# shadimsaleh/motion_detection

Measured on AMD Instinct MI355X. Metric: Mpixels/s (flow+warp+diff) at 1080p & 4K; % HBM roofline, 1/2/4/8 GPU, higher is better.
Workload: dtype u8

## Files before the change

motion_detection_amd/csrc/mdx_api.cpp:

```cpp
#include "mdx_ctx.h"

#include <cstdlib>
#include <map>
#include <mutex>

using namespace mdx;

static thread_local std::string g_create_err;

extern "C" void mdx_default_params(mdx_params* p)
{
    p->win = 40;
    p->max_level = 5;
    p->max_iters = 10;
    p->eps = 0.03;
    p->min_eig = 0.001f;
    p->thresh = 190;
    p->pixel_step = 10;
    p->min_vector_size = 1.0;
    p->fit_mode = MDX_FIT_FIRST4;
    p->subspace_precision = MDX_SUBSPACE_F64;
    p->call_pipelining = 0;
    p->ransac_iters = 128;
    p->ransac_thresh = 3.0;
    p->ransac_seed = 20141105u;
}

extern "C" int mdx_grid_count(int w, int h, int ps)
{
    if (w <= 0 || h <= 0 || ps <= 0) return 0;
    return ((w + ps - 1) / ps) * ((h + ps - 1) / ps);
}

static const char* check_params(const mdx_params* p)
{
    if (p->win != kWin) return "only win == 40 (the reference constant) is supported";
    if (p->max_level < 0 || p->max_level >= kMaxLevels) return "max_level out of range [0, 7]";
    if (p->pixel_step <= 0) return "pixel_step must be > 0 (reference leaves it unset: UB)";
    if (p->fit_mode != MDX_FIT_FIRST4 && p->fit_mode != MDX_FIT_EXTERNAL && p->fit_mode != MDX_FIT_RANSAC) return "bad fit_mode";
    if (p->ransac_iters < 1 || p->ransac_iters > kRansacMaxIters) return "ransac_iters must be in [1, 1024]";
    if (!(p->ransac_thresh >= 0.0) || !(p->ransac_thresh < 1e6)) return "ransac_thresh must be in [0, 1e6)";
    if (p->subspace_precision != MDX_SUBSPACE_F64 && p->subspace_precision != MDX_SUBSPACE_F32) return "bad subspace_precision";
    if (p->call_pipelining != 0 && p->call_pipelining != 1) return "call_pipelining must be 0 or 1";
    return nullptr;
}

static std::mutex g_host_mu;
static std::map<uintptr_t, size_t> g_host_blocks;
bool mdx::host_block_holds(const void* p, size_t bytes)
{
    const uintptr_t a = reinterpret_cast<uintptr_t>(p);
    std::lock_guard<std::mutex> lk(g_host_mu);
    auto it = g_host_blocks.upper_bound(a);
    if (it == g_host_blocks.begin()) return false;
    --it;
    return a >= it->first && bytes <= it->second && a - it->first <= it->second - bytes;
}

extern "C" const char* mdx_create_error(void) { return g_create_err.c_str(); }
extern "C" int mdx_abi_version(void) { return MDX_ABI_VERSION; }
extern "C" size_t mdx_params_size(void) { return sizeof(mdx_params); }

static LkTuning read_tuning()
{
    LkTuning t;
    auto num = [](const char* name, int dflt) {
        const char* e = std::getenv(name);
        return e ? std::atoi(e) : dflt;
    };
    t.lk_impl = num("MDX_LK_IMPL", 2) == 1 ? 1 : 2;
    t.lk_g = num("MDX_LK_G", 0);
    t.lk_sub = num("MDX_LK_SUB", 0);
    t.lk_astrip = std::max(0, std::min(num("MDX_LK_ASTRIP", 0), 64));
    t.lk_debug = num("MDX_LK_DEBUG", 0) != 0;
    t.traj_chain = num("MDX_TRAJ_CHAIN", 1) != 0;
    const int ppw = num("MDX_TRAJ_PPW", 4);
    t.traj_ppw = ppw == 1 ? 1 : ppw == 2 ? 2 : 4;
    t.lk_aux = num("MDX_LK_AUX", 1) != 0;
    t.lk_flow = num("MDX_LK_FLOW", 1) != 0;
    t.ol_reg = num("MDX_OL_REG", 1) != 0;
    t.lk_cap = std::min(std::max(num("MDX_LK_CAP", 75), 10), 100);
    t.lk_fma = num("MDX_LK_FMA", 1) != 0;
    t.spin_max = num("MDX_LK_SPIN_MAX", kLkSpinDefault);
    return t;
}

static bool new_stream(mdx_ctx* c, hipStream_t* s)
{
    if (hipStreamCreateWithFlags(s, hipStreamNonBlocking) != hipSuccess) {
        *s = nullptr;
        return false;
    }
    c->streams.push_back(*s);
    return true;
}

static bool new_events(mdx_ctx* c, hipEvent_t* e, int n, unsigned flags = hipEventDisableTiming)
{
    for (int i = 0; i < n; i++) {
        if (hipEventCreateWithFlags(&e[i], flags) != hipSuccess) return false;
        c->events.push_back(e[i]);
    }
    return true;
}

extern "C" mdx_ctx* mdx_create(int device, int max_w, int max_h, int max_batch, const mdx_params* p)
{
    g_create_err.clear();
    mdx_params prm;
    if (p) prm = *p;
    else mdx_default_params(&prm);
    if (const char* why = check_params(&prm)) { g_create_err = why; return nullptr; }
    if (max_w <= 0 || max_h <= 0 || max_batch <= 0) { g_create_err = "max_w/max_h/max_batch must be > 0"; return nullptr; }
    int ndev = 0;
    if (hipGetDeviceCount(&ndev) != hipSuccess || ndev == 0) { g_create_err = "no HIP device visible"; return nullptr; }
    if (device < 0 || device >= ndev) { g_create_err = "device index out of range"; return nullptr; }
    if (hipSetDevice(device) != hipSuccess) { g_create_err = "hipSetDevice failed"; return nullptr; }
    mdx_ctx* c = new mdx_ctx();
    c->device = device;
    c->prm = prm;
    c->max_w = max_w;
    c->max_h = max_h;
    c->max_batch = max_batch;
    static_cast<LkTuning&>(*c) = read_tuning();
    auto fail = [&](const std::string& msg) -> mdx_ctx* {
        g_create_err = msg;
        mdx_destroy(c);
        return nullptr;
    };
    if (!new_stream(c, &c->stream)) return fail("hipStreamCreate failed");
    if (c->lk_aux) {
        bool ok = new_stream(c, &c->aux) && new_events(c, c->lkev, kMaxLevels + 2);
        if (ok && c->lk_flow)
            ok = new_stream(c, &c->iter2) && new_events(c, c->flowev, 2) && new_events(c, c->redo_ev, kMaxLevels);
        ok = ok && new_events(c, &c->front_ev, 1) && new_events(c, c->pyr_free, 2) && new_events(c, c->lvl_done, kMaxLevels);
        if (!ok) return fail("aux stream / event creation failed");
    }
    c->lk = LkLaunch{c->stream, c->aux, c->iter2, c->lkev, c->flowev, c->iter2 ? c->redo_ev : nullptr};
    if (ensure(c, c->errw, 16) != MDX_OK || hipMemset(c->errw.p, 0, 16) != hipSuccess || !(c->err_host = pinned_ints(c, 4)))
        return fail("error-word allocation failed");
    Geometry g = make_geometry(max_w, max_h, prm.max_level);
    if (ensure_workspace(c, g, max_batch, prm.call_pipelining != 0) != MDX_OK) return fail(c->err);
    return c;
}

extern "C" int mdx_destroy(mdx_ctx* c)
{
    if (!c) return MDX_EINVAL;
    (void)hipSetDevice(c->device);
    for (hipStream_t s : {c->stream, c->aux, c->iter2})
        if (s) (void)hipStreamSynchronize(s);
    for (hipEvent_t e : c->events) (void)hipEventDestroy(e);
    for (hipStream_t s : c->streams) (void)hipStreamDestroy(s);
    for (void* p : c->pinned) (void)hipHostFree(p);
    delete c;
    return MDX_OK;
}

extern "C" const char* mdx_last_error(const mdx_ctx* c) { return c ? c->err.c_str() : "null context"; }
extern "C" void* mdx_stream(mdx_ctx* c) { return c ? (void*)c->stream : nullptr; }
extern "C" int mdx_device(const mdx_ctx* c) { return c ? c->device : -1; }
extern "C" int mdx_device_pci(const mdx_ctx* c, char* buf, int len)
{
    if (!c || !buf || len < 16) return MDX_EINVAL;
    return hipDeviceGetPCIBusId(buf, len, c->device) == hipSuccess ? MDX_OK : MDX_EHIP;
}

extern "C" int mdx_set_params(mdx_ctx* c, const mdx_params* p)
{
    if (!c || !p) return MDX_EINVAL;
    if (const char* why = check_params(p)) return set_err(c, MDX_EINVAL, "%s", why);
    c->prm = *p;
    return MDX_OK;
}

extern "C" int mdx_get_params(const mdx_ctx* c, mdx_params* p)
{
    if (!c || !p) return MDX_EINVAL;
    *p = c->prm;
    return MDX_OK;
}

static int lk_err_result(mdx_ctx* c)
{
    const int groups = c->err_host[0], gates = c->err_host[1], redone = c->err_host[2];
    if (groups == 0 && gates == 0 && redone == 0) return MDX_OK;
    c->err_host[0] = c->err_host[1] = c->err_host[2] = 0;
    c->lk_fallback[0] += groups;
    c->lk_fallback[1] += gates;
    c->lk_fallback[2] += redone;
    HIP_OR_RETURN(c, hipMemsetAsync(c->errw.p, 0, 12, c->stream));
    HIP_OR_RETURN(c, hipStreamSynchronize(c->stream));
    if (groups + gates > 0 && redone == 0)
        return set_err(c, MDX_EHIP, "LK dataflow: %d wait(s) and %d gate(s) gave up but no level was recomputed",
                       groups, gates);
    return MDX_OK;
}

extern "C" int mdx_lk_fallbacks(const mdx_ctx* c, long long* counts)
{
    if (!c || !counts) return MDX_EINVAL;
    for (int i = 0; i < 3; i++) counts[i] = c->lk_fallback[i];
    return MDX_OK;
}

static int sync_point(mdx_ctx* c, bool whole_device)
{
    if (!c) return MDX_EINVAL;
    HIP_OR_RETURN(c, hipSetDevice(c->device));
    HIP_OR_RETURN(c, hipMemcpyAsync(c->err_host, c->errw.p, 12, hipMemcpyDeviceToHost, c->stream));
    if (whole_device) HIP_OR_RETURN(c, hipDeviceSynchronize());
    else HIP_OR_RETURN(c, hipStreamSynchronize(c->stream));
    return lk_err_result(c);
}

extern "C" int mdx_sync(mdx_ctx* c) { return sync_point(c, false); }
extern "C" int mdx_device_sync(mdx_ctx* c) { return sync_point(c, true); }

extern "C" int mdx_input_ready(mdx_ctx* c, void* hip_event)
{
    if (!c) return MDX_EINVAL;
    c->input_ev = static_cast<hipEvent_t>(hip_event);
    return MDX_OK;
}

static constexpr int kSlots = 256;

extern "C" int mdx_enable_timing(mdx_ctx* c, int on)
{
    if (!c) return MDX_EINVAL;
    HIP_OR_RETURN(c, hipSetDevice(c->device));
    while (on && c->ev.size() < (size_t)kSlots * 7) {
        hipEvent_t e = nullptr;
        if (!new_events(c, &e, 1, hipEventDefault))
            return set_err(c, MDX_EHIP, "hipEventCreate(&c->ev[i]) failed: %s", hipGetErrorString(hipGetLastError()));
        c->ev.push_back(e);
    }
    c->timing = on != 0;
    c->ncalls = 0;
    c->cur = -1;
    return MDX_OK;
}

extern "C" int mdx_timing_calls(const mdx_ctx* c) { return c ? c->ncalls : 0; }

extern "C" int mdx_stage_ms(mdx_ctx* c, int stage, float* ms)
{
    if (!c || !ms || stage < 0 || stage > 6) return MDX_EINVAL;
    if (!c->timing || c->ev.empty()) return set_err(c, MDX_EINVAL, "timing not enabled");
    if (c->ncalls > kSlots) return set_err(c, MDX_EINVAL, "more than %d timed calls", kSlots);
    float total = 0.f;
    for (int k = 0; k < c->ncalls; k++) {
        hipEvent_t* e = c->ev.data() + k * 7;
        HIP_OR_RETURN(c, hipEventSynchronize(e[6]));
        float t = 0.f;
        if (stage == 6) HIP_OR_RETURN(c, hipEventElapsedTime(&t, e[0], e[6]));
        else HIP_OR_RETURN(c, hipEventElapsedTime(&t, e[stage], e[stage + 1]));
        total += t;
    }
    *ms = total;
    return MDX_OK;
}

#if MDX_WARP_STAMP
namespace mdx { hipError_t debug_warp_stamps(void* dst, size_t bytes); }
#endif
extern "C" int mdx_debug_copy(mdx_ctx* c, int which, void* dst, size_t bytes)
{
    if (!c || !dst) return MDX_EINVAL;
#if MDX_WARP_STAMP
    if (which == 99) {
        HIP_OR_RETURN(c, hipDeviceSynchronize());
        HIP_OR_RETURN(c, debug_warp_stamps(dst, bytes));
        return MDX_OK;
    }
#endif
    DevBuf& b = which == 0 ? c->Abuf : which == 1 ? c->dbg : which == 2 ? c->pyr1 : which == 3 ? c->pyr2
              : which == 4 ? c->der : which == 6 ? c->lkcnt : which == 7 ? c->sdata : which == 8 ? c->scnt : c->cls;
    if (!b.p) return set_err(c, MDX_EINVAL, "debug buffer %d unavailable", which);
    HIP_OR_RETURN(c, hipStreamSynchronize(c->stream));
    const uint8_t* src = static_cast<const uint8_t*>(b.p);
    if (which == 2 && c->last_pyr1) src = c->last_pyr1;
    if (which == 3 && c->last_pyr2) src = c->last_pyr2;
    const size_t avail = b.cap - (size_t)(src - static_cast<const uint8_t*>(b.p));
    HIP_OR_RETURN(c, hipMemcpy(dst, src, bytes < avail ? bytes : avail, hipMemcpyDeviceToHost));
    return MDX_OK;
}

extern "C" int mdx_debug_div32(mdx_ctx* c, const double* d_in, double* d_out, int n)
{
    if (!c || !d_in || !d_out || n <= 0) return MDX_EINVAL;
    HIP_OR_RETURN(c, hipSetDevice(c->device));
    HIP_OR_RETURN(c, launch_div32(c->stream, d_in, d_out, n));
    return MDX_OK;
}

extern "C" int mdx_debug_warp_paths(mdx_ctx* c, int32_t* out, int cap)
{
    if (!c || cap < 0 || (cap > 0 && !out)) return MDX_EINVAL;
    const WarpLaunch& L = c->last_warp;
    if (L.batch <= 0) return set_err(c, MDX_EINVAL, "mdx_debug_warp_paths: no warp launch on this context yet");
    HIP_OR_RETURN(c, hipSetDevice(c->device));
    HIP_OR_RETURN(c, debug_warp_paths(c->stream, L, out, cap));
    return L.batch * L.ntiles;
}

extern "C" void* mdx_host_alloc(size_t bytes)
{
    void* p = nullptr;
    if (hipHostMalloc(&p, bytes ? bytes : 1, hipHostMallocPortable) != hipSuccess) return nullptr;
    std::lock_guard<std::mutex> lk(g_host_mu);
    g_host_blocks[reinterpret_cast<uintptr_t>(p)] = bytes ? bytes : 1;
    return p;
}

extern "C" int mdx_host_free(void* p)
{
    if (!p) return MDX_OK;
    {
        std::lock_guard<std::mutex> lk(g_host_mu);
        g_host_blocks.erase(reinterpret_cast<uintptr_t>(p));
    }
    return hipHostFree(p) == hipSuccess ? MDX_OK : MDX_EHIP;
}

extern "C" void* mdx_dev_alloc(mdx_ctx* c, size_t bytes)
{
    if (!c) return nullptr;
    (void)hipSetDevice(c->device);
    void* p = nullptr;
    if (hipMalloc(&p, bytes ? bytes : 1) != hipSuccess) {
        set_err(c, MDX_ENOMEM, "hipMalloc(%zu) failed", bytes);
        return nullptr;
    }
    return p;
}

extern "C" int mdx_dev_free(mdx_ctx* c, void* p)
{
    if (!c) return MDX_EINVAL;
    (void)hipSetDevice(c->device);
    (void)hipStreamSynchronize(c->stream);
    HIP_OR_RETURN(c, hipFree(p));
    return MDX_OK;
}

extern "C" int mdx_memcpy_h2d(mdx_ctx* c, void* dst, const void* src, size_t bytes)
{
    if (!c) return MDX_EINVAL;
    HIP_OR_RETURN(c, hipMemcpyAsync(dst, src, bytes, hipMemcpyHostToDevice, c->stream));
    HIP_OR_RETURN(c, hipStreamSynchronize(c->stream));
    return MDX_OK;
}

extern "C" int mdx_memcpy_d2h(mdx_ctx* c, void* dst, const void* src, size_t bytes)
{
    if (!c) return MDX_EINVAL;
    HIP_OR_RETURN(c, hipMemcpyAsync(dst, src, bytes, hipMemcpyDeviceToHost, c->stream));
    HIP_OR_RETURN(c, hipStreamSynchronize(c->stream));
    return MDX_OK;
}

extern "C" int mdx_half_size(int w, int h, int* dw, int* dh)
{
    if (w < 2 || h < 2 || !dw || !dh) return MDX_EINVAL;
    auto half = [](int v) { return v / 2 + ((v & 1) & (v / 2 & 1)); };
    *dw = half(w);
    *dh = half(h);
    return MDX_OK;
}

static int check_half(mdx_ctx* c, const char* who, int batch, const uint8_t* src, int w, int h, int stride,
                      size_t frame_stride, int channels, const uint8_t* dst, int dst_stride, size_t dst_frame_stride,
                      int* dw, int* dh)
{
    if (!src || !dst || batch < 1) return set_err(c, MDX_EINVAL, "%s: null pointer or batch < 1", who);
    if (channels != 1 && channels != 3) return set_err(c, MDX_EINVAL, "%s: channels %d, not 1 or 3", who, channels);
    if (mdx_half_size(w, h, dw, dh) != MDX_OK) return set_err(c, MDX_EINVAL, "%s: a side of %d x %d halves to 0", who, w, h);
    if (*dh > 65535 * kHalfRows) return set_err(c, MDX_EINVAL, "%s: more than %d rows", who, 2 * 65535 * kHalfRows);
    if ((long long)w * channels > INT32_MAX || stride < w * channels)
        return set_err(c, MDX_EINVAL, "%s: stride %d < w*channels", who, stride);
    if (frame_stride < (size_t)h * (size_t)stride) return set_err(c, MDX_EINVAL, "%s: frame_stride < h*stride", who);
    if (dst_stride < *dw * channels) return set_err(c, MDX_EINVAL, "%s: dst_stride %d < dw*channels %d", who, dst_stride, *dw * channels);
    if (dst_frame_stride < (size_t)*dh * (size_t)dst_stride)
        return set_err(c, MDX_EINVAL, "%s: dst_frame_stride < dh*dst_stride", who);
    const uintptr_t s0 = reinterpret_cast<uintptr_t>(src), d0 = reinterpret_cast<uintptr_t>(dst);
    const uintptr_t s1 = s0 + (size_t)(batch - 1) * frame_stride + (size_t)(h - 1) * stride + (size_t)w * channels;
    const uintptr_t d1 = d0 + (size_t)(batch - 1) * dst_frame_stride + (size_t)(*dh - 1) * dst_stride + (size_t)*dw * channels;
    if (s0 < d1 && d0 < s1) return set_err(c, MDX_EINVAL, "%s: source and destination overlap", who);
    return MDX_OK;
}

extern "C" int mdx_resize_half_dev(mdx_ctx* c, int batch, const uint8_t* d_src, int w, int h, int stride,
                                   size_t frame_stride, int channels, uint8_t* d_dst, int dst_stride,
                                   size_t dst_frame_stride)
{
    if (!c) return MDX_EINVAL;
    int dw, dh;
    if (const int rc = check_half(c, "mdx_resize_half_dev", batch, d_src, w, h, stride, frame_stride, channels, d_dst,
                                  dst_stride, dst_frame_stride, &dw, &dh);
        rc != MDX_OK)
        return rc;
    HIP_OR_RETURN(c, hipSetDevice(c->device));
    hipStream_t s = c->stream;
    if (c->input_ev) {
        hipEvent_t e = c->input_ev;
        c->input_ev = nullptr;
        HIP_OR_RETURN(c, hipStreamWaitEvent(s, e, 0));
    }
    HIP_OR_RETURN(c, launch_half(s, batch, d_src, w, h, stride, frame_stride, channels, d_dst, dst_stride, dst_frame_stride));
    return MDX_OK;
}

extern "C" int mdx_resize_half(mdx_ctx* c, const uint8_t* src, int w, int h, int stride, int channels, uint8_t* dst,
                               int dst_stride)
{
    if (!c) return MDX_EINVAL;
    int dw, dh;
    const size_t fs = (size_t)std::max(h, 0) * (size_t)std::max(stride, 0);
    if (const int rc = check_half(c, "mdx_resize_half", 1, src, w, h, stride, fs, channels, dst, dst_stride,
                                  (size_t)std::max(h, 0) * (size_t)std::max(dst_stride, 0), &dw, &dh);
        rc != MDX_OK)
        return rc;
    HIP_OR_RETURN(c, hipSetDevice(c->device));
    const int dpitch = (dw * channels + 3) & ~3;
    if (const int rc = ensure_all(c, {{&c->hsrc, fs}, {&c->hdst, (size_t)dpitch * dh}}); rc != MDX_OK) return rc;
    hipStream_t s = c->stream;
    HIP_OR_RETURN(c, hipMemcpyAsync(c->hsrc.p, src, (size_t)(h - 1) * stride + (size_t)w * channels, hipMemcpyHostToDevice, s));
    HIP_OR_RETURN(c, launch_half(s, 1, c->hsrc.as<uint8_t>(), w, h, stride, 0, channels, c->hdst.as<uint8_t>(), dpitch, 0));
    HIP_OR_RETURN(c, hipMemcpy2DAsync(dst, (size_t)dst_stride, c->hdst.p, (size_t)dpitch, (size_t)dw * channels, (size_t)dh,
                                      hipMemcpyDeviceToHost, s));
    HIP_OR_RETURN(c, hipStreamSynchronize(s));
    return MDX_OK;
}
```

motion_detection_amd/csrc/mdx_ctx.h:

```cpp
#pragma once

#include "../../include/mdx.h"
#include "mdx_internal.h"

#include <algorithm>
#include <array>
#include <cstdarg>
#include <cstdio>
#include <initializer_list>
#include <string>
#include <utility>
#include <vector>

struct DevBuf {
    void* p = nullptr;
    size_t cap = 0;
    DevBuf() = default;
    DevBuf(DevBuf&& o) noexcept : p(std::exchange(o.p, nullptr)), cap(std::exchange(o.cap, 0)) {}
    DevBuf& operator=(DevBuf&& o) noexcept
    {
        std::swap(p, o.p), std::swap(cap, o.cap);
        return *this;
    }
    ~DevBuf() { reset(); }
    void reset()
    {
        if (p) (void)hipFree(p);
        p = nullptr, cap = 0;
    }
    bool alloc(size_t bytes)
    {
        reset();
        if (hipMalloc(&p, bytes) != hipSuccess) p = nullptr;
        cap = p ? bytes : 0;
        return p != nullptr;
    }
    template <typename T> T* as() const { return static_cast<T*>(p); }
};

struct LkTuning {
    int lk_impl = 2;
    int lk_g = 0;
    int lk_sub = 0;
    int lk_astrip = 0;
    bool lk_debug = false;
    bool traj_chain = true;
    int traj_ppw = 4;
    bool lk_aux = true;
    bool lk_flow = true;
    int lk_cap = 75;
    bool lk_fma = true;
    int spin_max = mdx::kLkSpinDefault;
    bool ol_reg = true;
};

struct mdx_ctx : LkTuning {
    int device = 0;
    std::vector<hipStream_t> streams;
    std::vector<hipEvent_t> events;
    std::vector<void*> pinned;
    hipStream_t stream = nullptr;
    hipStream_t aux = nullptr;
    hipEvent_t lkev[mdx::kMaxLevels + 2] = {};
    hipStream_t iter2 = nullptr;
    hipEvent_t flowev[2] = {};
    hipEvent_t front_ev = nullptr;
    hipEvent_t pyr_free[2] = {};
    hipEvent_t lvl_done[mdx::kMaxLevels] = {};
    hipEvent_t redo_ev[mdx::kMaxLevels] = {};
    mdx::LkLaunch lk;
    int pyr_half = 0;
    hipEvent_t input_ev = nullptr;
    uint8_t* last_pyr1 = nullptr;
    uint8_t* last_pyr2 = nullptr;
    uint8_t* band_pyr1 = nullptr;
    uint8_t* band_pyr2 = nullptr;
    int band_half = 0;
    const uint8_t* band_img1 = nullptr;
    int band_built[2] = {0, 0};
    int band_stride = 0, band_fmt = 0;
    DevBuf errw;
    int* err_host = nullptr;
    int* tcnt_host = nullptr;
    long long lk_fallback[3] = {0, 0, 0};
    mdx_params prm{};
    int max_w = 0, max_h = 0, max_batch = 0;
    DevBuf pyr1, pyr2, der, fits;
    DevBuf in1, in2, np, st, vec, mask, H, Hext, num;
    DevBuf bnp, bst;
    DevBuf cls, Abuf, ctab;
    DevBuf dbg;
    DevBuf lkcnt;
    DevBuf csum;
    DevBuf tin, tcur, tnp, tst, ttraj, tnum, tflag;
    DevBuf straj, sdata, sq, scnt, scols, sres, sout, sbest;
    DevBuf clpts, clbest, clroot;
    std::vector<int32_t> cl_host;
    DevBuf vcpts, vcroot, vcrows, vcq;
    std::vector<double> vc_host;
    std::vector<float> vc_pts;
    std::vector<int32_t> vc_idx;
    DevBuf olin, olmag, olout;
    std::vector<double> ol_host;
    std::vector<uint8_t> ol_flags;
    DevBuf rgscr;
    DevBuf rgin, rgout;
    DevBuf ring_pyr, ring_der, rin;
    DevBuf rfull;
    DevBuf hsrc, hdst;
    DevBuf wscr;
    mdx::WarpLaunch last_warp;
    DevBuf rsc;
    std::vector<int> ring_order;
    int ring_cap = 0, ring_w = 0, ring_h = 0, ring_ml = -1;
    std::array<size_t, 4> lk_scratch_key{{0, 0, 0, 0}};
    std::array<int, 6> plan_key{{-1, -1, -1, -1, -1, -1}};
    int band_w = 0, band_h = 0;
    mdx::ClassPlan plan{};
    bool timing = false;
    std::vector<hipEvent_t> ev;
    int ncalls = 0;
    int cur = -1;
    std::string err;
};

namespace mdx {

inline int set_err(mdx_ctx* c, int code, const char* fmt, ...)
{
    char buf[512];
    va_list ap;
    va_start(ap, fmt);
    vsnprintf(buf, sizeof(buf), fmt, ap);
    va_end(ap);
    if (c) c->err = buf;
    return code;
}

#define HIP_OR_RETURN(c, expr)                                                                 \
    do {                                                                                       \
        hipError_t e_ = (expr);                                                                \
        if (e_ != hipSuccess)                                                                  \
            return set_err((c), MDX_EHIP, "%s failed: %s", #expr, hipGetErrorString(e_));      \
    } while (0)

inline Geometry make_geometry(int w, int h, int max_level)
{
    Geometry g{};
    int sw = w, sh = h;
    long long img = 0, der = 0;
    int lvl;
    for (lvl = 0; lvl <= max_level; lvl++) {
        Level& L = g.lv[lvl];
        L.w = sw;
        L.h = sh;
        L.pitch = (kXOff + sw + kPad + 16 + 63) / 64 * 64;
        L.rows = kPad + sh + kPad;
        L.img_off = img;
        L.der_off = der;
        img += (long long)L.pitch * L.rows;
        der += (long long)L.pitch * L.rows;
        g.nlev = lvl + 1;
        sw = (sw + 1) / 2;
        sh = (sh + 1) / 2;
        if (sw <= kWin || sh <= kWin) break;
    }
    g.img_bytes = (img + 255) / 256 * 256;
    g.der_words = (der + 63) / 64 * 64;
    return g;
}

inline int ensure(mdx_ctx* c, DevBuf& b, size_t need)
{
    if (need == 0) need = 1;
    if (b.p && b.cap >= need) return MDX_OK;
    if (b.p) (void)hipStreamSynchronize(c->stream);
    if (!b.alloc(need)) return set_err(c, MDX_ENOMEM, "hipMalloc(%zu) failed", need);
    return MDX_OK;
}

inline int* pinned_ints(mdx_ctx* c, int n)
{
    void* p = nullptr;
    if (hipHostMalloc(&p, sizeof(int) * n, hipHostMallocDefault) != hipSuccess) return nullptr;
    c->pinned.push_back(p);
    return static_cast<int*>(p);
}

inline int ensure_all(mdx_ctx* c, std::initializer_list<std::pair<DevBuf*, size_t>> needs)
{
    for (const auto& n : needs)
        if (const int rc = ensure(c, *n.first, n.second); rc != MDX_OK) return rc;
    return MDX_OK;
}

inline size_t slab_slack_bytes(const Geometry& g) { return ((size_t)g.lv[g.nlev - 1].pitch + 255) / 256 * 256; }

inline size_t pyr_half_bytes(const DevBuf& b) { return b.cap / 2 / 256 * 256; }

inline int ensure_workspace(mdx_ctx* c, const Geometry& g, int batch, bool two)
{
    const size_t half = ((size_t)g.img_bytes * batch + 255) / 256 * 256 + slab_slack_bytes(g);
    return ensure_all(c, {{&c->pyr1, two ? 2 * half : half}, {&c->pyr2, two ? 2 * half : half},
                          {&c->der, (size_t)g.der_words * 4 * batch}, {&c->fits, sizeof(PairFit) * (size_t)batch}});
}

inline int check_frame(mdx_ctx* c, const char* who, int w, int h, int stride, int fmt)
{
    const char* sep = who ? ": " : "";
    if (!who) who = "";
    if (w <= 0 || h <= 0) return set_err(c, MDX_EINVAL, "%s%sbad frame size", who, sep);
    if (fmt < MDX_FMT_GRAY8 || fmt > MDX_FMT_BGR8) return set_err(c, MDX_EINVAL, "%s%sbad pixel format %d", who, sep, fmt);
    const int cn = fmt == MDX_FMT_GRAY8 ? 1 : 3;
    if (stride < w * cn) return set_err(c, MDX_EINVAL, "%s%sstride %d < w*channels %d", who, sep, stride, w * cn);
    return MDX_OK;
}

inline size_t frame_copy_bytes(int w, int h, int stride, int fmt)
{
    const int cn = fmt == MDX_FMT_GRAY8 ? 1 : 3;
    return (size_t)stride * (size_t)(h - 1) + (size_t)w * cn;
}

inline LkArgs lk_args_for(const mdx_ctx* c, const Geometry& g, int w, int h)
{
    const mdx_params& P = c->prm;
    LkArgs a{};
    a.g = g;
    a.maxl = g.nlev - 1;
    a.npts = mdx_grid_count(w, h, P.pixel_step);
    a.ny = (h + P.pixel_step - 1) / P.pixel_step;
    a.nyg = a.ny;
    a.pixel_step = P.pixel_step;
    a.max_iters = std::min(std::max(P.max_iters, 0), 100);
    a.min_eig = P.min_eig;
    const double e = std::min(std::max(P.eps, 0.), 10.);
    a.eps2 = e * e;
    return a;
}

inline void release_pyr_all(mdx_ctx* c)
{
    for (hipEvent_t e : c->pyr_free)
        if (e) (void)hipEventRecord(e, c->stream);
}

int run_lk(mdx_ctx* c, const Geometry& g, LkArgs& a, int batch, int w, int h, int gy0, int gy1, bool have_scharr,
           hipEvent_t prev_ready = nullptr);
bool host_block_holds(const void* p, size_t bytes);

}
```

motion_detection_amd/csrc/mdx_internal.h:

```cpp
#pragma once

#include <hip/hip_runtime.h>
#include <math.h>
#include <stdint.h>

#include <algorithm>

#include "mdx.h"

namespace mdx {

constexpr int kMaxLevels = 8;
constexpr int kLkDbgStampOff = kMaxLevels * 64 + 64;
constexpr int kLkDbgWaves = 16384;
constexpr int kWin = 40;
constexpr int kPad = 40;
constexpr int kXOff = 64;

struct Level {
    int w, h;
    int pitch;
    int rows;
    long long img_off;
    long long der_off;
    __host__ __device__ long long core() const { return (long long)kPad * pitch + kXOff; }
};

struct Geometry {
    int nlev;
    Level lv[kMaxLevels];
    long long img_bytes;
    long long der_words;
};
inline uint8_t* level0_core(uint8_t* slab, const Geometry& g) { return slab + g.lv[0].img_off + g.lv[0].core(); }

struct PairFit {
    double H[9];
    double Hinv[9];
    int num_vectors;
    int fit_status;
    int src_y0, src_y1;
};

struct ClassLevel {
    int nrx, nry;
    int UH, PW;
    long long off;
    long long class_bytes;
    int nxp;
    int ord_off;
    int G;
    int UW;
    int vlo, vhi;
    int asp;
    int nstrip;
    int strip_off;
};
constexpr int kAStripRows = 16;

__host__ __device__ inline int lk_win_origin(int gi, int pixel_step, int level)
{
    return (int)floorf((float)(gi * pixel_step) * (float)(1. / (1 << level)) - 19.5f);
}
__host__ __device__ inline int lk_win_row0(int ipy, int UH) { return std::min(std::max(ipy + kPad, 0), UH - kWin); }

#define LK_SHAPES LK_CASE(4, 48) LK_CASE(4, 56) LK_CASE(4, 64) LK_CASE(4, 72) LK_CASE(4, 80) LK_CASE(4, 96) \
    LK_CASE(4, 128) LK_CASE(8, 80) LK_CASE(8, 112) LK_CASE(8, 128) LK_CASE(8, 256) LK_CASE(8, 512)
constexpr int kLkUW4[] = {48, 56, 64, 72, 80, 96, 128};
constexpr int kLkUW8[] = {80, 112, 128, 256, 512};

struct ClassPlan {
    ClassLevel lv[kMaxLevels];
    long long bytes_per_pair;
    int nch;
};

struct LkClassArgs {
    Geometry g;
    ClassPlan plan;
    const int16_t* rlist;
    int level;
};

struct LkArgs {
    const uint8_t* pyr1;
    const uint8_t* pyr2;
    const uint32_t* der;
    Geometry g;
    int maxl;
    int npts, ny, pixel_step;
    int nyg;
    int max_iters;
    float min_eig;
    double eps2;
    float* next_pts;
    float* carry;
    long long carry_lstride;
    uint8_t* status;
    ClassPlan plan;
    const int16_t* cmap;
    const int16_t* rlist;
    const int16_t* ord;
    const float* prev_pts;
    int max_sub;
    int* done;
    int done_stride;
    int dep_groups;
    int* err;
    int* lflags;
    int redo;
    int spin_max;
    int flow_cap;
    float4* dbg;
    int dbg_pt;
    int fma;
    uint32_t* body_cnt;
};

constexpr int kCtrPad = 32;
constexpr int kLkSpinDefault = 1 << 19;
constexpr int kLkFlagGiveup = 0;
constexpr int kLkFlagRedone = kMaxLevels;
constexpr int kLkFlagQueue = 2 * kMaxLevels;
constexpr int kLkFlagInts = kLkFlagQueue + 8 * kMaxLevels;
#ifndef MDX_LK_REDO_WAVES
#define MDX_LK_REDO_WAVES 512
#endif
constexpr int kLkRedoWaves = MDX_LK_REDO_WAVES;

struct RowSpan {
    int lo, hi;
};

hipError_t launch_gray_pad(hipStream_t s, int batch, const uint8_t* in1, const uint8_t* in2, int w, int h,
                           int stride, long long frame_stride, int fmt, uint8_t* pyr1, uint8_t* pyr2,
                           const Geometry& g, int fsel = 0);
hipError_t launch_front(hipStream_t s, int batch, const uint8_t* in1, const uint8_t* in2, int w, int h, int stride,
                        long long frame_stride, int fmt, uint8_t* pyr1, uint8_t* pyr2, const Geometry& g,
                        int fsel = 0, const RowSpan* rows = nullptr);
hipError_t launch_pyr_levels(hipStream_t s, int batch, uint8_t* pyr1, uint8_t* pyr2, const Geometry& g, int fsel = 0,
                             const RowSpan* rows = nullptr);
hipError_t launch_scharr_levels(hipStream_t s, int batch, const uint8_t* pyr1, uint32_t* der, const Geometry& g);
hipError_t launch_scharr(hipStream_t s, int batch, const uint8_t* pyr1, uint32_t* der, const Geometry& g, int level,
                         int prow0 = 0, int prow1 = -1);
hipError_t launch_lk(hipStream_t s, int batch, const LkArgs& a);

constexpr int kMaxTrajImgs = 16;
struct TrajChain {
    const uint8_t* pyr[kMaxTrajImgs];
    const uint32_t* der[kMaxTrajImgs];
    int nimg, w, h;
    float* cur;
    float* traj;
    int* tlen;
    int* flag;
    double* vectors;
    float* start_pts;
    int* num;
    double mvs;
    float* htraj;
    int* htlen;
    float* hstart;
    double* hvec;
};
hipError_t launch_lk_chain(hipStream_t s, const LkArgs& a, const TrajChain& t, int ppw);
hipError_t launch_subspace(hipStream_t s, const float* traj, int N, int T, int d, const int* cols, int nhyp,
                           double sigma, float* data, double* qbuf, int* counts, double* residuals,
                           uint8_t* is_outlier, int* best, int precision);
constexpr int kClB = 256;
hipError_t launch_cluster(hipStream_t s, const float* pts, int N, uint32_t slim, unsigned long long* best,
                          int32_t* root);
size_t vcluster_rows_bytes(int nA);
hipError_t launch_vcluster(hipStream_t s, const double* xyt, int nA, double slim, double athr, int abs_int,
                           uint32_t* rows, uint32_t* qscan, uint32_t* cand, int32_t* root);
hipError_t launch_outliers(hipStream_t s, int batch, int n, const double* dxy, double* ang, double* mag,
                           int include_zeros, uint8_t* flags, mdx_outlier_stats* stats, bool in_registers);
hipError_t launch_traj_init(hipStream_t s, int npts, int ny, int pixel_step, int nimg, float* cur, float* traj,
                            int* tlen, int* num, int* flag = nullptr);
hipError_t launch_traj_update(hipStream_t s, int npts, const float* next_pts, const uint8_t* status, float* cur,
                              float* traj, int* tlen, int nimg, int w, int h, int last, double min_vector_size,
                              double* vectors, float* start_pts, int* num);
struct LkLaunch {
    hipStream_t s = nullptr;
    hipStream_t aux = nullptr;
    hipStream_t s2 = nullptr;
    hipEvent_t* ev = nullptr;
    hipEvent_t* flow_ev = nullptr;
    hipEvent_t* redo_ev = nullptr;
    uint8_t* cls = nullptr;
    float4* Ab = nullptr;
    uint8_t* cert = nullptr;
    int* qctr = nullptr;
    int* done = nullptr;
    hipEvent_t* lvl_done = nullptr;
    hipEvent_t prev_ready = nullptr;
};
hipError_t launch_lk_v2(const LkLaunch& L, int batch, const LkArgs& a);
constexpr int kRansacMaxIters = 1024;
struct RansacArgs {
    int iters;
    double thresh;
    uint32_t seed;
    int* list;
    double* hyps;
    int* counts;
};
struct RansacScratch {
    size_t hyps, counts, bytes;
};
inline RansacScratch ransac_scratch(int batch, int npts, int iters)
{
    const size_t list_b = (size_t)batch * npts * sizeof(int), hyps_b = (size_t)batch * iters * 9 * sizeof(double),
                 counts_b = (size_t)batch * iters * sizeof(int);
    RansacScratch L;
    L.hyps = (list_b + 7) & ~(size_t)7;
    L.counts = L.hyps + hyps_b;
    L.bytes = list_b + hyps_b + counts_b + 256;
    return L;
}
inline size_t ransac_scratch_bytes(int batch, int npts, int iters) { return ransac_scratch(batch, npts, iters).bytes; }
inline RansacArgs ransac_args(void* base, int batch, int npts, const mdx_params& P)
{
    const RansacScratch L = ransac_scratch(batch, npts, P.ransac_iters);
    uint8_t* b = static_cast<uint8_t*>(base);
    return {P.ransac_iters, P.ransac_thresh, P.ransac_seed, reinterpret_cast<int*>(b),
            reinterpret_cast<double*>(b + L.hyps), reinterpret_cast<int*>(b + L.counts)};
}
struct BlockSummary {
    int count;
    int first[4];
    int ransac_off;
    int pad_[2];
};
static_assert(sizeof(BlockSummary) == 32, "BlockSummary: eight ints, two records per 64-B line");
inline int classify_blocks(int npts) { return (npts + 255) / 256; }
inline size_t classify_scratch_bytes(int batch, int npts)
{
    return (size_t)batch * classify_blocks(npts) * sizeof(BlockSummary);
}
struct FitArgs {
    const float* next_pts;
    const uint8_t* status;
    int npts, ny, pixel_step;
    int gy0, gy1;
    double min_vector_size;
    double* vectors;
    PairFit* fits;
    int fit_mode;
    const double* H_external;
    void* scratch;
    mdx_band_cand* cand;
    RansacArgs ransac;
};
hipError_t launch_classify_fit(hipStream_t s, int batch, const FitArgs& a);
hipError_t launch_band_fit(hipStream_t s, int nrec, const mdx_band_cand* cands, PairFit* fit, int w, int h, int y0,
                           int y1);
hipError_t launch_gray_rows(hipStream_t s, const uint8_t* img1, int w, int h, int stride, int fmt, uint8_t* gray1_l0,
                            int pitch, const PairFit* fit, int built0 = 0, int built1 = 0);
hipError_t launch_set_fit_external(hipStream_t s, int batch, const double* H_external, PairFit* fits);
size_t warp_scratch_bytes(int batch, int w, int rows);
struct WarpLaunch {
    int batch = 0, ntiles = 0;
    int bw0 = 0, vec_ok = 0;
    const PairFit* fits = nullptr;
    const void* tinfo = nullptr;
};
struct GrayPlane {
    const uint8_t* p;
    long long frame_stride;
    int pitch;
};
struct WarpArgs {
    GrayPlane g1, g2;
    int w, h;
    const PairFit* fits;
    uint8_t* mask;
    long long mask_stride;
    int thresh;
    int row0 = 0, row1 = -1;
};
hipError_t launch_warp_diff(hipStream_t s, int batch, const WarpArgs& a, void* scratch, size_t scratch_bytes,
                            WarpLaunch* rec = nullptr);
hipError_t debug_warp_paths(hipStream_t s, const WarpLaunch& L, int32_t* out, int cap);
hipError_t launch_div32(hipStream_t s, const double* in, double* out, int n);
hipError_t launch_stream3(hipStream_t s, size_t n, const uint8_t* a, const uint8_t* b, uint8_t* o, int thresh);
hipError_t launch_export_fit(hipStream_t s, int batch, const PairFit* fits, double* H, int* num_vectors);
constexpr int kRegionsMaxBatch = 65535;
struct RegionsScratch {
    size_t lab, blk, stats, nall;
};
size_t regions_scratch_bytes(int batch, int w, int h, RegionsScratch* lay = nullptr);
hipError_t launch_mask_regions(hipStream_t s, int batch, const uint8_t* mask, int w, int h, int stride,
                               size_t frame_stride, int open3, int min_area, mdx_region* regions, int max_regions,
                               int32_t* num_all, int32_t* num_kept, int32_t* labels, uint8_t* mask_out, void* scratch);

constexpr int kHalfPx = 4;
constexpr int kHalfWavePx = 64 * kHalfPx;
constexpr int kHalfWgPx = 256 * kHalfPx;
constexpr int kHalfRows = 4;
constexpr int kHalfMaxBatch = 65535;
bool half_vector_path(int batch, const void* src, int stride, size_t frame_stride, const void* dst, int dst_stride,
                      size_t dst_frame_stride);
hipError_t launch_half(hipStream_t s, int batch, const uint8_t* src, int w, int h, int stride, size_t frame_stride,
                       int channels, uint8_t* dst, int dst_stride, size_t dst_frame_stride);

}
```

motion_detection_amd/csrc/mdx_lk.hip:

```cpp
#include "mdx_internal.h"

#include <float.h>

#include <algorithm>
#include <atomic>
#include <cstdlib>
#include <type_traits>

namespace mdx {

typedef short s2 __attribute__((ext_vector_type(2)));
typedef float f2 __attribute__((ext_vector_type(2)));
struct __attribute__((aligned(4))) u2a4 { uint32_t x, y; };
struct __attribute__((aligned(4))) u3a4 { uint32_t x, y, z; };
typedef unsigned int v4u __attribute__((ext_vector_type(4)));
typedef unsigned int v3u __attribute__((ext_vector_type(3)));
__device__ __forceinline__ __amdgpu_buffer_rsrc_t buf_rsrc(const void* base, long long bytes)
{
    return __builtin_amdgcn_make_buffer_rsrc(const_cast<void*>(base), (short)0,
                                             (int)min(bytes, (long long)0x7fffffff), 0x00020000);
}
__device__ __forceinline__ __amdgpu_buffer_rsrc_t buf_rsrc32(const void* base, uint32_t bytes)
{
    const unsigned long long b = (unsigned long long)(uintptr_t)base;
    const uint32_t lo = __builtin_amdgcn_readfirstlane((uint32_t)b), hi = __builtin_amdgcn_readfirstlane((uint32_t)(b >> 32));
    void* p = (void*)(uintptr_t)(((unsigned long long)hi << 32) | lo);
    return __builtin_amdgcn_make_buffer_rsrc(p, (short)0, (int)__builtin_amdgcn_readfirstlane(bytes), 0x00020000);
}

__device__ __forceinline__ int class_of(const int16_t* cmap, int level, int axis, int res)
{
    return cmap[(level * 2 + axis) * 128 + res];
}
__device__ __forceinline__ int residue_of(const int16_t* rlist, int level, int axis, int cls)
{
    return rlist[(level * 2 + axis) * 128 + cls];
}

__device__ __forceinline__ void lk_weights(float fa, float fb, int& w00, int& w01, int& w10, int& w11)
{
    w00 = __float2int_rn((1.f - fa) * (1.f - fb) * 16384.f);
    w01 = __float2int_rn(fa * (1.f - fb) * 16384.f);
    w10 = __float2int_rn((1.f - fa) * fb * 16384.f);
    w11 = 16384 - w00 - w01 - w10;
}

template <int Q>
__device__ __forceinline__ void lk_interp(uint32_t lo0, uint32_t hi0, uint32_t lo1, uint32_t hi1, uint32_t d00,
                                          uint32_t d01, uint32_t d10, uint32_t d11, s2 W0, s2 W1, int& ival, int& ixv,
                                          int& iyv)
{
    static_assert(Q >= 0 && Q < 7, "tap byte");
    constexpr unsigned sel = 0x0c000c00u | (unsigned)Q | ((unsigned)(Q + 1) << 16);
    const s2 t0 = __builtin_bit_cast(s2, __builtin_amdgcn_perm(hi0, lo0, sel));
    const s2 t1 = __builtin_bit_cast(s2, __builtin_amdgcn_perm(hi1, lo1, sel));
    ival = __builtin_amdgcn_sdot2(t0, W0, __builtin_amdgcn_sdot2(t1, W1, 256, false), false) >> 9;
    const s2 x0 = __builtin_bit_cast(s2, __builtin_amdgcn_perm(d01, d00, 0x05040100u));
    const s2 x1 = __builtin_bit_cast(s2, __builtin_amdgcn_perm(d11, d10, 0x05040100u));
    const s2 y0 = __builtin_bit_cast(s2, __builtin_amdgcn_perm(d01, d00, 0x07060302u));
    const s2 y1 = __builtin_bit_cast(s2, __builtin_amdgcn_perm(d11, d10, 0x07060302u));
    ixv = __builtin_amdgcn_sdot2(x0, W0, __builtin_amdgcn_sdot2(x1, W1, 8192, false), false) >> 14;
    iyv = __builtin_amdgcn_sdot2(y0, W0, __builtin_amdgcn_sdot2(y1, W1, 8192, false), false) >> 14;
}

template <int J>
__device__ __forceinline__ float quad_bcast(float v)
{
    constexpr int ctrl = J | (J << 2) | (J << 4) | (J << 6);
    return __int_as_float(__builtin_amdgcn_mov_dpp(__float_as_int(v), ctrl, 0xf, 0xf, false));
}
template <int J>
__device__ __forceinline__ uint32_t quad_bcast_u(uint32_t v)
{
    constexpr int ctrl = J | (J << 2) | (J << 4) | (J << 6);
    return (uint32_t)__builtin_amdgcn_mov_dpp((int)v, ctrl, 0xf, 0xf, false);
}

__device__ __forceinline__ void wave_lds_fence()
{
    __builtin_amdgcn_fence(__ATOMIC_RELEASE, "wavefront");
    __builtin_amdgcn_wave_barrier();
    __builtin_amdgcn_fence(__ATOMIC_ACQUIRE, "wavefront");
}

constexpr int kLkIterWavesPerEU = 4;
typedef __attribute__((address_space(3))) void* lds_ptr;
typedef __attribute__((address_space(3))) uint32_t lds_u32;
typedef unsigned int v2u __attribute__((ext_vector_type(2)));
typedef __attribute__((address_space(3))) volatile const v2u lds_u2v;
typedef __attribute__((address_space(3))) volatile const v4u lds_u4v;
__device__ __forceinline__ void lk_vmcnt0()
{
    __builtin_amdgcn_sched_barrier(0);
    __builtin_amdgcn_s_waitcnt(0x0F70);
    __builtin_amdgcn_sched_barrier(0);
}
template <int N>
__device__ __forceinline__ void lk_vmcnt()
{
    static_assert(N >= 0 && N < 16, "vmcnt field");
    __builtin_amdgcn_sched_barrier(0);
    __builtin_amdgcn_s_waitcnt(0x0F70 | N);
    __builtin_amdgcn_sched_barrier(0);
}

template <int B, int E, typename F>
__device__ __forceinline__ void static_for(F&& f)
{
    if constexpr (B < E) {
        f(std::integral_constant<int, B>{});
        static_for<B + 1, E>(f);
    }
}

__device__ __forceinline__ int xcd_remap(int b, int total)
{
    const int xcd = b & 7, q = total >> 3, r = total & 7;
    return (xcd < r ? xcd * (q + 1) : r * (q + 1) + (xcd - r) * q) + (b >> 3);
}

__device__ __forceinline__ void cls_store(uint4* o, const uint32_t (&dv)[4], const int (&cv)[4])
{
    typedef unsigned v4nt __attribute__((ext_vector_type(4)));
    const uint4 a = make_uint4(dv[0], (uint32_t)cv[0], dv[1], (uint32_t)cv[1]);
    const uint4 b = make_uint4(dv[2], (uint32_t)cv[2], dv[3], (uint32_t)cv[3]);
    __builtin_nontemporal_store(__builtin_bit_cast(v4nt, a), reinterpret_cast<v4nt*>(o));
    __builtin_nontemporal_store(__builtin_bit_cast(v4nt, b), reinterpret_cast<v4nt*>(o) + 1);
}

__global__ __launch_bounds__(256) void k_lk_class(const uint8_t* __restrict__ pyr1, const uint32_t* __restrict__ der,
                                                  uint8_t* __restrict__ cls_out, LkClassArgs a)
{
    const int level = a.level;
    const ClassLevel& C = a.plan.lv[level];
    const int nclass = C.nrx * C.nry;
    const int pair = blockIdx.z / nclass, cls = blockIdx.z % nclass;
    const int j = blockIdx.x * blockDim.x + threadIdx.x;
    const int v = C.vlo + blockIdx.y;
    if (4 * j >= a.g.lv[level].w + 2 * kPad || v >= C.UH) return;
    const Level L = a.g.lv[level];
    const float scale = (float)(1. / (1 << level));
    const int rx = residue_of(a.rlist, level, 0, cls % C.nrx), ry = residue_of(a.rlist, level, 1, cls / C.nrx);
    const float ppx = (float)rx * scale - 19.5f, ppy = (float)ry * scale - 19.5f;
    const float fa = ppx - floorf(ppx), fb = ppy - floorf(ppy);
    int w00, w01, w10, w11;
    lk_weights(fa, fb, w00, w01, w10, w11);
    const uint8_t* I = pyr1 + (long long)pair * a.g.img_bytes + L.img_off + L.core();
    const uint32_t* D = der + (long long)pair * a.g.der_words + L.der_off + L.core();
    const int y = v - kPad;
    const int p = L.pitch;
    uint8_t* base = cls_out + (long long)pair * a.plan.bytes_per_pair + C.off + (long long)cls * C.class_bytes;
    uint32_t dv[4] = {0, 0, 0, 0};
    int cv[4];
    const int x0 = 4 * j - kPad;
    if (y < L.h + kPad - 1 && x0 < L.w + kPad - 1) {
        const uint8_t* ip = I + (long long)y * p + x0;
        const uint32_t* dp = D + (long long)y * p + x0;
        uint32_t ib[2][2], dw[2][5];
#pragma unroll
        for (int r = 0; r < 2; r++) {
            const u2a4 bi = *reinterpret_cast<const u2a4*>(ip + (long long)r * p);
            ib[r][0] = bi.x; ib[r][1] = bi.y;
            const uint4 d4 = *reinterpret_cast<const uint4*>(dp + (long long)r * p);
            dw[r][0] = d4.x; dw[r][1] = d4.y; dw[r][2] = d4.z; dw[r][3] = d4.w;
            dw[r][4] = dp[(long long)r * p + 4];
        }
        const s2 W0 = {(short)w00, (short)w01}, W1 = {(short)w10, (short)w11};
        static_for<0, 4>([&](auto qc) {
            constexpr int q = decltype(qc)::value;
            if (x0 + q >= L.w + kPad - 1) { cv[q] = 256; return; }
            int ival, ixv, iyv;
            lk_interp<q>(ib[0][0], ib[0][1], ib[1][0], ib[1][1], dw[0][q], dw[0][q + 1], dw[1][q], dw[1][q + 1], W0, W1,
                         ival, ixv, iyv);
            dv[q] = ((uint32_t)ixv & 0xffffu) | ((uint32_t)iyv << 16);
            cv[q] = 256 - 512 * ival;
        });
    } else {
#pragma unroll
        for (int q = 0; q < 4; q++) cv[q] = 256;
    }
    uint4* o = reinterpret_cast<uint4*>(base) + ((long long)v * C.PW + 4 * j) / 2;
    cls_store(o, dv, cv);
}

__device__ __forceinline__ int u8_at(const uint32_t (&w)[3], int b) { return (int)((w[b >> 2] >> (8 * (b & 3))) & 255u); }

__global__ __launch_bounds__(256) void k_lk_class_fused(const uint8_t* __restrict__ pyr1, uint8_t* __restrict__ cls_out,
                                                        LkClassArgs a)
{
    const int level = a.level;
    const ClassLevel& C = a.plan.lv[level];
    const int nclass = C.nrx * C.nry;
    const int pair = blockIdx.z;
    const int j = blockIdx.x * blockDim.x + threadIdx.x;
    const int v = C.vlo + blockIdx.y;
    if (4 * j >= a.g.lv[level].w + 2 * kPad || v >= C.UH) return;
    const Level L = a.g.lv[level];
    const float scale = (float)(1. / (1 << level));
    const uint8_t* I = pyr1 + (long long)pair * a.g.img_bytes + L.img_off + L.core();
    const int y = v - kPad;
    const int p = L.pitch;
    const int x0 = 4 * j - kPad;
    const bool inside = y < L.h + kPad - 1 && x0 < L.w + kPad - 1;
    uint32_t rw[4][3];
#pragma unroll
    for (int r = 0; r < 4; r++) {
        const int yy = y - 1 + r;
        const int ys = (yy < -kPad || yy >= L.h + kPad) ? y : yy;
        const u3a4 t = *reinterpret_cast<const u3a4*>(I + (long long)ys * p + x0 - 4);
        rw[r][0] = t.x; rw[r][1] = t.y; rw[r][2] = t.z;
    }
    uint32_t dw[2][5];
#pragma unroll
    for (int r = 0; r < 2; r++) {
        const int yy = y + r;
#pragma unroll
        for (int c = 0; c < 5; c++) {
            const int x = x0 + c;
            uint32_t d = 0;
            if (yy >= 0 && yy < L.h && x >= 0 && x < L.w) {
                const int bm = 3 + c, bc = 4 + c, bp = 5 + c;
                const int t0m = (u8_at(rw[r], bm) + u8_at(rw[r + 2], bm)) * 3 + u8_at(rw[r + 1], bm) * 10;
                const int t0p = (u8_at(rw[r], bp) + u8_at(rw[r + 2], bp)) * 3 + u8_at(rw[r + 1], bp) * 10;
                const int t1m = u8_at(rw[r + 2], bm) - u8_at(rw[r], bm), t1c = u8_at(rw[r + 2], bc) - u8_at(rw[r], bc);
                const int t1p = u8_at(rw[r + 2], bp) - u8_at(rw[r], bp);
                const int ix = t0p - t0m, iy = (t1m + t1p) * 3 + t1c * 10;
                d = (uint32_t)(uint16_t)(int16_t)ix | ((uint32_t)(uint16_t)(int16_t)iy << 16);
            }
            dw[r][c] = d;
        }
    }
    for (int cls = 0; cls < nclass; cls++) {
        const int rx = residue_of(a.rlist, level, 0, cls % C.nrx), ry = residue_of(a.rlist, level, 1, cls / C.nrx);
        const float ppx = (float)rx * scale - 19.5f, ppy = (float)ry * scale - 19.5f;
        const float fa = ppx - floorf(ppx), fb = ppy - floorf(ppy);
        int w00, w01, w10, w11;
        lk_weights(fa, fb, w00, w01, w10, w11);
        uint32_t dv[4] = {0, 0, 0, 0};
        int cv[4] = {256, 256, 256, 256};
        if (inside) {
            const s2 W0 = {(short)w00, (short)w01}, W1 = {(short)w10, (short)w11};
            static_for<0, 4>([&](auto qc) {
                constexpr int q = decltype(qc)::value;
                if (x0 + q >= L.w + kPad - 1) return;
                int ival, ixv, iyv;
                lk_interp<q>(rw[1][1], rw[1][2], rw[2][1], rw[2][2], dw[0][q], dw[0][q + 1], dw[1][q], dw[1][q + 1], W0,
                             W1, ival, ixv, iyv);
                dv[q] = ((uint32_t)ixv & 0xffffu) | ((uint32_t)iyv << 16);
                cv[q] = 256 - 512 * ival;
            });
        }
        uint8_t* base = cls_out + (long long)pair * a.plan.bytes_per_pair + C.off + (long long)cls * C.class_bytes;
        uint4* o = reinterpret_cast<uint4*>(base) + ((long long)v * C.PW + 4 * j) / 2;
        cls_store(o, dv, cv);
    }
}

template <int G, int UW>
struct LkShape {
    static constexpr int UWIDTH = UW;
    static constexpr int LPS = 4 * G;
    static constexpr int S = 64 / LPS;
    static constexpr int NP = (UW + 2 * LPS - 1) / (2 * LPS);
    static constexpr int BYTES = S * UW * 8;
    static constexpr int ND = (BYTES + 1023) / 1024;
    static_assert(UW % 2 == 0 && UW >= kWin, "union width");
};

struct GroupGeom {
    int gx, gy;
    bool valid;
    int ipx, ipy;
    int off;
    int v0;
    uint32_t ubase;
};

template <int G, int UW>
__device__ __forceinline__ GroupGeom group_geom(const LkArgs& a, const ClassLevel& C, int level, int g, int sl)
{
    GroupGeom r;
    const int16_t* xo = a.ord + C.ord_off;
    const int16_t* yo = xo + C.nxp;
    const bool has = g >= 0;
    const int gg = has ? g : 0;
    const int cg = gg / a.nyg, row = gg - cg * a.nyg;
    const int e0 = cg * G;
    const int gxv = has ? xo[e0 + (sl >> 2)] : -1;
    r.valid = gxv >= 0;
    r.gx = r.valid ? gxv : 0;
    r.gy = yo[row];
    r.ipx = lk_win_origin(r.gx, a.pixel_step, level);
    r.ipy = lk_win_origin(r.gy, a.pixel_step, level);
    const int gx0 = has ? xo[e0] : 0;
    const int ipx0 = lk_win_origin(gx0, a.pixel_step, level);
    const int m = (1 << level) - 1;
    const int cx = class_of(a.cmap, level, 0, (gx0 * a.pixel_step) & m);
    const int cy = class_of(a.cmap, level, 1, (r.gy * a.pixel_step) & m);
    const int ub = min(max(ipx0 + kPad, 0), C.PW - UW);
    r.off = min(max(r.ipx + kPad - ub, 0), UW - kWin);
    r.v0 = lk_win_row0(r.ipy, C.UH);
    r.ubase = (uint32_t)(C.off + (long long)(cy * C.nrx + cx) * C.class_bytes) + 8u * (uint32_t)ub;
    return r;
}

template <typename Sh>
__device__ __forceinline__ void lk_piece_offsets(uint32_t mine, int lane, uint32_t (&uoff)[Sh::ND])
{
#pragma unroll
    for (int c = 0; c < Sh::ND; c++) {
        const int P = 1024 * c + 16 * lane;
        const int sp = P / (8 * Sh::UWIDTH), wb = P % (8 * Sh::UWIDTH);
        uoff[c] = (uint32_t)__shfl((int)mine, sp * Sh::LPS) + (uint32_t)wb;
    }
}

template <typename Sh>
struct LkRowImages {
    lds_u32 *img0, *img1, *img2;
    __amdgpu_buffer_rsrc_t crs;
    uint32_t rowb;

    template <int B>
    __device__ __forceinline__ lds_u32* ibuf() const
    {
        if constexpr (B == 0) return img0;
        else if constexpr (B == 1) return img1;
        else return img2;
    }
    __device__ __forceinline__ void mask_past(int lane, uint32_t (&uoff)[Sh::ND]) const
    {
#pragma unroll
        for (int c = 0; c < Sh::ND; c++)
            if (1024 * c + 16 * lane >= Sh::BYTES) uoff[c] = 0x80000000u;
    }
    template <int B>
    __device__ __forceinline__ void dma(uint32_t (&uoff)[Sh::ND]) const
    {
        lds_u32* I = ibuf<B>();
#pragma unroll
        for (int c = 0; c < Sh::ND; c++) {
            __builtin_amdgcn_raw_ptr_buffer_load_lds(crs, (lds_ptr)(I + 256 * c), 16, (int)uoff[c], 0, 0, 0);
            uoff[c] += rowb;
        }
    }
};

__device__ __forceinline__ float4 lk_A_result(f2 sd, float s12, bool ok, float min_eig)
{
    constexpr float FLT_SCALE = 1.f / (1 << 20);
    const float a11 = ((quad_bcast<0>(sd.x) + quad_bcast<1>(sd.x)) + quad_bcast<2>(sd.x)) + quad_bcast<3>(sd.x);
    const float a12 = ((quad_bcast<0>(s12) + quad_bcast<1>(s12)) + quad_bcast<2>(s12)) + quad_bcast<3>(s12);
    const float a22 = ((quad_bcast<0>(sd.y) + quad_bcast<1>(sd.y)) + quad_bcast<2>(sd.y)) + quad_bcast<3>(sd.y);
    const float A11 = a11 * FLT_SCALE, A12 = a12 * FLT_SCALE, A22 = a22 * FLT_SCALE;
    float Dinv = 0.f;
    if (ok) {
        const float D = A11 * A22 - A12 * A12;
        const float minEig = (A22 + A11 - __builtin_sqrtf((A11 - A22) * (A11 - A22) + 4.f * A12 * A12)) /
                             (float)(2 * kWin * kWin);
        if (!(minEig < min_eig || D < FLT_EPSILON)) Dinv = 1.f / D;
    }
    return make_float4(A11, A12, A22, Dinv);
}

constexpr float kLkCertMax = 2056.f;
static_assert(kLkCertMax * 8160.f < 16777216.f, "certified products are exact in float");
__device__ __forceinline__ float lk_mag_max(float m, f2 f)
{
    return __builtin_fmaxf(__builtin_fmaxf(m, __builtin_fabsf(f.x)), __builtin_fabsf(f.y));
}
__device__ __forceinline__ f2 lk_fma(f2 f, float fd, f2 acc) { return __builtin_elementwise_fma(f, f2{fd, fd}, acc); }
__device__ __forceinline__ uint8_t lk_cert_flag(float m)
{
    const float q = __builtin_fmaxf(__builtin_fmaxf(quad_bcast<0>(m), quad_bcast<1>(m)),
                                    __builtin_fmaxf(quad_bcast<2>(m), quad_bcast<3>(m)));
    return q <= kLkCertMax ? 1 : 0;
}

template <int G, int UW>
__global__ __launch_bounds__(64) void k_lk_A(LkArgs a, const uint8_t* __restrict__ cls, float4* __restrict__ Ab,
                                             uint8_t* __restrict__ cert, int* __restrict__ qctr, int level, int ngroups)
{
    using Sh = LkShape<G, UW>;
    constexpr int LPS = Sh::LPS, S = Sh::S, ND = Sh::ND;
    constexpr int NB = 3;
    __shared__ __attribute__((aligned(16))) uint32_t img0[ND * 256];
    __shared__ __attribute__((aligned(16))) uint32_t img1[ND * 256];
    __shared__ __attribute__((aligned(16))) uint32_t img2[ND * 256];

    const int lane = threadIdx.x, k = lane & 3, slot = lane / LPS, sl = lane % LPS;
    const int nw = gridDim.x;
    const int bid = xcd_remap(blockIdx.x + nw * blockIdx.y, nw * gridDim.y);
    const int pair = bid / nw, w = bid % nw;
    if (bid == 0 && lane < 8) qctr[(level * 8 + lane) * kCtrPad] = 0;
    const ClassLevel& C = a.plan.lv[level];
    const Level L = a.g.lv[level];
    const int g = w * S + slot;
    const GroupGeom q = group_geom<G, UW>(a, C, level, g < ngroups ? g : -1, sl);
    bool ok = q.valid && !(q.ipx < -kWin || q.ipx >= L.w || q.ipy < -kWin || q.ipy >= L.h);

    LkRowImages<Sh> im{(lds_u32*)img0, (lds_u32*)img1, (lds_u32*)img2,
                       buf_rsrc(cls + (long long)pair * a.plan.bytes_per_pair, a.plan.bytes_per_pair),
                       (uint32_t)C.PW * 8};
    uint32_t uoff[ND];
    lk_piece_offsets<Sh>(q.ubase + (uint32_t)q.v0 * im.rowb, lane, uoff);
    im.mask_past(lane, uoff);
    const int el = 2 * (slot * UW + q.off + k);

    f2 sd = {0.f, 0.f};
    float s12 = 0.f, mag = 0.f;
    constexpr int PF = NB - 1;
    im.template dma<0>(uoff);
    im.template dma<1>(uoff);
    static_for<0, kWin>([&](auto yc) {
        constexpr int y = decltype(yc)::value;
        constexpr int later = (y + PF - 1 < kWin - 1 ? y + PF - 1 : kWin - 1) - y;
        lk_vmcnt<later * ND>();
        if constexpr (y + PF < kWin) im.template dma<(y + PF) % NB>(uoff);
        __builtin_amdgcn_sched_barrier(0);
        lds_u2v* lE = (lds_u2v*)(im.template ibuf<y % NB>() + el);
        uint32_t dw[10];
#pragma unroll
        for (int gi = 0; gi < 10; gi++) dw[gi] = lE[4 * gi].x;
#pragma unroll
        for (int gi = 0; gi < 10; gi++) {
            const uint32_t d = dw[gi];
            const f2 f = {(float)(int16_t)d, (float)((int)d >> 16)};
            sd = __builtin_elementwise_fma(f, f, sd);
            s12 = __builtin_fmaf(f.x, f.y, s12);
            mag = lk_mag_max(mag, f);
        }
        asm volatile("" : "+v"(mag));
    });
    const float4 r = lk_A_result(sd, s12, ok, a.min_eig);
    const uint8_t cf = lk_cert_flag(mag);
    if (q.valid && k == 0) {
        Ab[(long long)pair * a.npts + q.gx * a.ny + q.gy] = r;
        cert[(long long)pair * a.npts + q.gx * a.ny + q.gy] = cf;
    }
}

template <int G, int UW, int NW>
__global__ __launch_bounds__(64) void k_lk_A_rows(LkArgs a, const uint8_t* __restrict__ cls, float4* __restrict__ Ab,
                                                  uint8_t* __restrict__ cert, int* __restrict__ qctr, int level, int ncg)
{
    using Sh = LkShape<G, UW>;
    constexpr int LPS = Sh::LPS, S = Sh::S, ND = Sh::ND;
    __shared__ __attribute__((aligned(16))) uint32_t img0[ND * 256];
    __shared__ __attribute__((aligned(16))) uint32_t img1[ND * 256];
    __shared__ __attribute__((aligned(16))) uint32_t img2[ND * 256];

    const int lane = threadIdx.x, k = lane & 3, slot = lane / LPS, sl = lane % LPS;
    const int nw = gridDim.x;
    const int bid = xcd_remap(blockIdx.x + nw * blockIdx.y, nw * gridDim.y);
    const int pair = bid / nw, w = bid % nw;
    if (bid == 0 && lane < 8) qctr[(level * 8 + lane) * kCtrPad] = 0;
    const ClassLevel& C = a.plan.lv[level];
    const Level L = a.g.lv[level];
    const int ncw = (ncg + S - 1) / S;
    const int strip = w / ncw, cg = (w - strip * ncw) * S + slot;
    const int16_t* xo = a.ord + C.ord_off;
    const int16_t* yo = xo + C.nxp;
    const int r0 = a.ord[C.strip_off + 2 * strip], nr = a.ord[C.strip_off + 2 * strip + 1];
    const int asp = C.asp;
    const int m = (1 << level) - 1;
    const int gx0 = cg < ncg ? xo[cg * G] : -1;
    const int gxv = cg < ncg ? xo[cg * G + (sl >> 2)] : -1;
    const bool valid = gxv >= 0;
    const int gx = valid ? gxv : 0;
    const int ipx = lk_win_origin(gx, a.pixel_step, level);
    const int gy0 = yo[r0];
    const int ipx0 = lk_win_origin(gx0 >= 0 ? gx0 : 0, a.pixel_step, level);
    const int cx = class_of(a.cmap, level, 0, ((gx0 >= 0 ? gx0 : 0) * a.pixel_step) & m);
    const int cy = class_of(a.cmap, level, 1, (gy0 * a.pixel_step) & m);
    const int ub = min(max(ipx0 + kPad, 0), C.PW - UW);
    const int off = min(max(ipx + kPad - ub, 0), UW - kWin);
    const uint32_t ubase = (uint32_t)(C.off + (long long)(cy * C.nrx + cx) * C.class_bytes) + 8u * (uint32_t)ub;
    const int v00 = lk_win_row0(lk_win_origin(gy0, a.pixel_step, level), C.UH);
    const int R = (nr - 1) * asp + kWin;

    LkRowImages<Sh> im{(lds_u32*)img0, (lds_u32*)img1, (lds_u32*)img2,
                       buf_rsrc(cls + (long long)pair * a.plan.bytes_per_pair, a.plan.bytes_per_pair),
                       (uint32_t)C.PW * 8};
    uint32_t uoff[ND];
    lk_piece_offsets<Sh>(ubase + (uint32_t)v00 * im.rowb, lane, uoff);
    im.mask_past(lane, uoff);
    const int el = 2 * (slot * UW + off + k);

    static_assert(NW % 2 == 0, "slot pairs");
    typedef unsigned short us2 __attribute__((ext_vector_type(2)));
    f2 sd[NW];
    float s12[NW];
    us2 magp[NW / 2];
    int rin[NW], jw[NW];
#pragma unroll
    for (int s = 0; s < NW / 2; s++) magp[s] = us2{0, 0};
#pragma unroll
    for (int s = 0; s < NW; s++) {
        sd[s] = f2{0.f, 0.f};
        s12[s] = 0.f;
        rin[s] = -1;
        jw[s] = 0;
    }
    int nextj = 0;
    auto finish = [&](int j, f2 sdv, float s12v, float magv) {
        const int gy = yo[r0 + j];
        const int ipy = lk_win_origin(gy, a.pixel_step, level);
        const bool ok = valid && !(ipx < -kWin || ipx >= L.w || ipy < -kWin || ipy >= L.h);
        const float4 r = lk_A_result(sdv, s12v, ok, a.min_eig);
        const uint8_t cf = lk_cert_flag(magv);
        if (valid && k == 0) {
            Ab[(long long)pair * a.npts + gx * a.ny + gy] = r;
            cert[(long long)pair * a.npts + gx * a.ny + gy] = cf;
        }
    };
    auto row = [&](int t, auto bc) {
        if (t + 1 < R) lk_vmcnt<ND>();
        else lk_vmcnt0();
        constexpr int B = decltype(bc)::value;
        if (t + 2 < R) im.template dma<(B + 2) % 3>(uoff);
        __builtin_amdgcn_sched_barrier(0);
        lds_u2v* lE = (lds_u2v*)(im.template ibuf<B>() + el);
        uint32_t dw[10];
#pragma unroll
        for (int gi = 0; gi < 10; gi++) dw[gi] = lE[4 * gi].x;
        f2 f[10];
#pragma unroll
        for (int gi = 0; gi < 10; gi++) f[gi] = f2{(float)(int16_t)dw[gi], (float)((int)dw[gi] >> 16)};
        float rmag = 0.f;
#pragma unroll
        for (int gi = 0; gi < 10; gi++) rmag = lk_mag_max(rmag, f[gi]);
        if (nextj < nr && t == nextj * asp) {
            static_for<0, NW>([&](auto sc) {
                constexpr int s = decltype(sc)::value;
                if (nextj % NW == s) {
                    sd[s] = f2{0.f, 0.f};
                    s12[s] = 0.f;
                    magp[s / 2][s & 1] = 0;
                    rin[s] = 0;
                    jw[s] = nextj;
                }
            });
            nextj++;
        }
        const unsigned short ri = (unsigned short)(uint32_t)rmag;
#pragma unroll
        for (int s = 0; s < NW / 2; s++) magp[s] = __builtin_elementwise_max(magp[s], us2{ri, ri});
        static_for<0, NW>([&](auto sc) {
            constexpr int s = decltype(sc)::value;
            if (rin[s] >= 0) {
#pragma unroll
                for (int gi = 0; gi < 10; gi++) {
                    sd[s] = __builtin_elementwise_fma(f[gi], f[gi], sd[s]);
                    s12[s] = __builtin_fmaf(f[gi].x, f[gi].y, s12[s]);
                }
                if (++rin[s] == kWin) {
                    finish(jw[s], sd[s], s12[s], (float)magp[s / 2][s & 1]);
                    rin[s] = -1;
                }
            }
        });
    };
    im.template dma<0>(uoff);
    if (R > 1) im.template dma<1>(uoff);
#pragma unroll 1
    for (int t = 0; t < R; t += 3) {
        row(t, std::integral_constant<int, 0>{});
        if (t + 1 < R) row(t + 1, std::integral_constant<int, 1>{});
        if (t + 2 < R) row(t + 2, std::integral_constant<int, 2>{});
    }
}

template <int G, int UW, bool DF>
__global__ __launch_bounds__(64) __attribute__((amdgpu_waves_per_eu(kLkIterWavesPerEU, 8))) void k_lk_iter(
    LkArgs a, const uint8_t* __restrict__ cls, const float4* __restrict__ Ab, const uint8_t* __restrict__ cert,
    int* __restrict__ qctr, int level, int ngroups, int batch)
{
    using Sh = LkShape<G, UW>;
    constexpr int LPS = Sh::LPS, S = Sh::S, ND = Sh::ND;
    constexpr float HALFW = 19.5f;
    constexpr float FLT_SCALE = 1.f / (1 << 20);
    constexpr int UB = S * UW;
    static_assert(kWin % 2 == 0, "row schedule (row pairs)");
    __shared__ __attribute__((aligned(16))) uint32_t dU0[2 * UB];
    __shared__ __attribute__((aligned(16))) uint32_t dU1[2 * UB];
    __shared__ __attribute__((aligned(16))) uint32_t dJ0[256];
    __shared__ __attribute__((aligned(16))) uint32_t dJ1[256];

    const int lane = threadIdx.x, k = lane & 3, slot = lane / LPS, sl = lane % LPS;
    const unsigned long long smask = ((1ull << LPS) - 1) << (slot * LPS);
    const unsigned long long t_start = a.dbg ? __builtin_amdgcn_s_memrealtime() : 0ull;
    const int xcd = blockIdx.x & 7;
    int* const a_done = DF ? a.done : nullptr;
    int* const a_lflags = DF ? a.lflags : nullptr;
    const int a_redo = DF ? a.redo : 0;
    const int dep_groups = DF ? a.dep_groups : 0;
    const long long T = (long long)batch * ngroups;
    const long long cb = T * xcd / 8, ce = T * (xcd + 1) / 8;
    const int p0 = (int)(cb / ngroups);
    const uint32_t off0 = (uint32_t)(cb - (long long)p0 * ngroups);
    const int np = ce > cb ? (int)((ce - 1) / ngroups) - p0 + 1 : 1;
    int* ctr = qctr + (level * 8 + xcd) * kCtrPad;
    if (a_redo) {
        int need = __hip_atomic_load(a_lflags + (kLkFlagGiveup + level) * kCtrPad, __ATOMIC_RELAXED,
                                     __HIP_MEMORY_SCOPE_AGENT);
        if (level < a.maxl)
            need |= __hip_atomic_load(a_lflags + (kLkFlagRedone + level + 1) * kCtrPad, __ATOMIC_RELAXED,
                                      __HIP_MEMORY_SCOPE_AGENT);
        if (!need) return;
        if (blockIdx.x == 0 && lane == 0) {
            __hip_atomic_store(a_lflags + (kLkFlagRedone + level) * kCtrPad, 1, __ATOMIC_RELAXED,
                               __HIP_MEMORY_SCOPE_AGENT);
            __hip_atomic_fetch_add(a.err + 2, 1, __ATOMIC_RELAXED, __HIP_MEMORY_SCOPE_AGENT);
        }
        ctr = a_lflags + (kLkFlagQueue + level * 8 + xcd) * kCtrPad;
    }
    int* const giveup = a_lflags ? a_lflags + (kLkFlagGiveup + level) * kCtrPad : nullptr;
    const ClassLevel& C = a.plan.lv[level];
    const Level L = a.g.lv[level];
    const uint8_t* const cls_base = cls + (long long)p0 * a.plan.bytes_per_pair;
    const uint32_t cls_bytes = (uint32_t)(np * a.plan.bytes_per_pair);
    const uint32_t rowb = (uint32_t)C.PW * 8;
    const int pitch = L.pitch;
    const uint8_t* const j_base = a.pyr2 + (long long)p0 * a.g.img_bytes;
    const uint32_t j_bytes = (uint32_t)(np * a.g.img_bytes);
    const uint32_t jbase = (uint32_t)(L.img_off + L.core());
    const float scale = (float)(1. / (1 << level));

    bool live = false, dead = false;
    int j = 0;
    GroupGeom q{};
    int pt = 0, pair = 0;
    long long po = 0;
    uint32_t jrel = 0;
    float A11 = 0.f, A12 = 0.f, A22 = 0.f, Dinv = 0.f;
    float nx = 0.f, ny = 0.f, npx = 0.f, npy = 0.f, pdx = 0.f, pdy = 0.f;
    bool act = false, gave_up = false;
    bool certd = false;
    int status = 1, iters = 0;
    uint32_t n_exact = 0, n_fused = 0;

    auto retire = [&]() {
        if (level == 0 && q.valid && status) {
            const int fx = (int)floorf(npx - HALFW), fy = (int)floorf(npy - HALFW);
            if (fx < -kWin || fx >= L.w || fy < -kWin || fy >= L.h) status = 0;
        }
        if (q.valid && k == 0) {
            if (a.dbg)
                a.dbg[((long long)pair * a.g.nlev + level) * a.npts + pt] = make_float4(npx, npy, (float)iters, (float)status);
            const float2 v = make_float2(npx, npy);
            float* dst = (a.carry && level > 0) ? a.carry + level * a.carry_lstride : a.next_pts;
            if (a_done)
                __hip_atomic_store(reinterpret_cast<unsigned long long*>(dst) + po,
                                   __builtin_bit_cast(unsigned long long, v), __ATOMIC_RELAXED, __HIP_MEMORY_SCOPE_AGENT);
            else
                reinterpret_cast<float2*>(dst)[po] = v;
            if (level == 0) a.status[po] = (uint8_t)status;
        }
        if (a_done && level > 0) {
            asm volatile("s_waitcnt vmcnt(0)" ::: "memory");
            if (sl == 0)
                __hip_atomic_fetch_add(a_done + (level * a.done_stride + pair) * kCtrPad, 1, __ATOMIC_RELAXED,
                                       __HIP_MEMORY_SCOPE_AGENT);
        }
    };

    for (;;) {
        for (;;) {
            const bool need = !live && !dead;
            if (!__any(need)) break;
            if (need) {
                int gi = 0;
                if (sl == 0) gi = atomicAdd(ctr, 1);
                gi = __shfl(gi, slot * LPS);
                if (cb + gi >= ce) {
                    dead = true;
                } else {
                    const uint32_t r = off0 + (uint32_t)gi, dp = r / (uint32_t)ngroups;
                    pair = p0 + (int)dp;
                    q = group_geom<G, UW>(a, C, level, (int)(r - dp * (uint32_t)ngroups), sl);
                    q.ubase += (uint32_t)((long long)(pair - p0) * a.plan.bytes_per_pair);
                    jrel = (uint32_t)((long long)(pair - p0) * a.g.img_bytes);
                    pt = q.gx * a.ny + q.gy;
                    po = (long long)pair * a.npts + pt;
                    const float4 Av = q.valid ? Ab[po] : make_float4(0.f, 0.f, 0.f, 0.f);
                    A11 = Av.x;
                    A12 = Av.y;
                    A22 = Av.z;
                    Dinv = Av.w;
                    certd = q.valid && cert[po] != 0;
                    if (level == a.maxl) {
                        npx = (float)(q.gx * a.pixel_step) * scale;
                        npy = (float)(q.gy * a.pixel_step) * scale;
                    } else {
                        float2 p = make_float2(0.f, 0.f);
                        const float* src = a.carry ? a.carry + (level + 1) * a.carry_lstride : a.next_pts;
                        if (dep_groups) {
                            if (sl == 0 && !gave_up) {
                                const int* d = a_done + ((level + 1) * a.done_stride + pair) * kCtrPad;
                                int slept = 0, gap = 1;
                                bool mine = false;
                                if (a.spin_max < 0) mine = true;
                                while (!mine &&
                                       __hip_atomic_load(d, __ATOMIC_RELAXED, __HIP_MEMORY_SCOPE_AGENT) < dep_groups) {
                                    if (slept >= a.spin_max) {
                                        mine = true;
                                        break;
                                    }
                                    if (__hip_atomic_load(giveup, __ATOMIC_RELAXED, __HIP_MEMORY_SCOPE_AGENT) > 0) {
                                        gave_up = true;
                                        break;
                                    }
                                    for (int i = 0; i < gap; i++) __builtin_amdgcn_s_sleep(8);
                                    slept += gap;
                                    gap = gap < 16 ? 2 * gap : 16;
                                }
                                if (mine) {
                                    gave_up = true;
                                    __hip_atomic_fetch_add(giveup, 1, __ATOMIC_RELAXED, __HIP_MEMORY_SCOPE_AGENT);
                                    __hip_atomic_fetch_add(a.err, 1, __ATOMIC_RELAXED, __HIP_MEMORY_SCOPE_AGENT);
                                }
                            }
                            __builtin_amdgcn_fence(__ATOMIC_ACQUIRE, "wavefront");
                            if (q.valid)
                                p = __builtin_bit_cast(float2, __hip_atomic_load(reinterpret_cast<const unsigned long long*>(src) + po,
                                                                                 __ATOMIC_RELAXED, __HIP_MEMORY_SCOPE_AGENT));
                        } else if (q.valid) {
                            p = reinterpret_cast<const float2*>(src)[po];
                        }
                        npx = p.x * 2.f;
                        npy = p.y * 2.f;
                    }
                    act = Dinv > 0.f;
                    if (dep_groups && (__ballot(gave_up) & smask)) act = false;
                    status = (level == 0 && q.valid && !act) ? 0 : 1;
                    nx = npx - HALFW;
                    ny = npy - HALFW;
                    pdx = 0.f;
                    pdy = 0.f;
                    iters = 0;
                    j = 0;
                    live = (__ballot(act) & smask) != 0 && a.max_iters > 0;
                    if (!live) retire();
                }
            }
        }
        if (!__any(live)) break;

        f2 acc = {0.f, 0.f};
        if (act) iters++;
        int inx = (int)floorf(nx), iny = (int)floorf(ny);
        if (act && (inx < -kWin || inx >= L.w || iny < -kWin || iny >= L.h)) {
            act = false;
            if (level == 0) status = 0;
        }
        if (!act) { inx = 0; iny = 0; }
        const float fa = nx - (float)inx, fb = ny - (float)iny;
        int v00, v01, v10, v11;
        lk_weights(fa, fb, v00, v01, v10, v11);
        const s2 W0 = {(short)v00, (short)v01};
        const s2 W1 = {(short)v10, (short)v11};
        const int o = (inx & 3) + k;
        const unsigned sel = (unsigned)o | 0x0c00u | ((unsigned)(o + 1) << 16) | 0x0c000000u;
        uint32_t joff = jrel + jbase + (uint32_t)(iny * pitch + (inx & ~3) + 16 * k);
        uint32_t uoff[ND];
        lk_piece_offsets<Sh>(q.ubase + (uint32_t)q.v0 * rowb, lane, uoff);
        auto ubuf = [&](auto bc) -> uint32_t* {
            if constexpr (decltype(bc)::value == 0) return dU0;
            else return dU1;
        };
        auto jbuf = [&](auto bc) -> uint32_t* {
            if constexpr (decltype(bc)::value == 0) return dJ0;
            else return dJ1;
        };
        auto dma_union = [&](auto bc, int yr) {
            uint32_t* U = ubuf(bc);
            const uint32_t adv = (uint32_t)yr * rowb;
            const __amdgpu_buffer_rsrc_t r = buf_rsrc32(cls_base + adv, cls_bytes - adv);
#pragma unroll
            for (int c = 0; c < ND; c++) {
                if (c < ND - 1 || 1024 * c + 16 * lane < Sh::BYTES)
                    __builtin_amdgcn_raw_ptr_buffer_load_lds(r, (lds_ptr)(U + 256 * c), 16, (int)uoff[c], 0, 0, 0);
            }
        };
        auto dma_j = [&](auto bc, int yr) {
            const uint32_t adv = (uint32_t)(yr * pitch);
            const __amdgpu_buffer_rsrc_t r = buf_rsrc32(j_base + adv, j_bytes - adv);
            if (k < 3) __builtin_amdgcn_raw_ptr_buffer_load_lds(r, (lds_ptr)jbuf(bc), 16, (int)joff, 0, 0, 0);
        };
        const int jl = (lane >> 2) * 16, el = 2 * (slot * UW + q.off + k);
        auto read_j = [&](auto bc, uint32_t (&rj)[11]) {
            lds_u4v* lJ = (lds_u4v*)(jbuf(bc) + jl);
            const v4u j0 = lJ[0], j1 = lJ[1], j2 = lJ[2];
            rj[0] = j0.x; rj[1] = j0.y; rj[2] = j0.z; rj[3] = j0.w;
            rj[4] = j1.x; rj[5] = j1.y; rj[6] = j1.z; rj[7] = j1.w;
            rj[8] = j2.x; rj[9] = j2.y; rj[10] = j2.z;
        };
        using I0 = std::integral_constant<int, 0>;
        using I1 = std::integral_constant<int, 1>;
        s2 pa[10], pb[10];
        dma_union(I0{}, 0);
        dma_j(I0{}, 0);
        dma_j(I1{}, 1);
        lk_vmcnt0();
        {
            uint32_t rj[11];
            read_j(I0{}, rj);
#pragma unroll
            for (int gi = 0; gi < 10; gi++) pa[gi] = __builtin_bit_cast(s2, __builtin_amdgcn_perm(rj[gi + 1], rj[gi], sel));
        }
        auto row = [&](auto Fc, int y, auto Rc, s2 (&up)[10], s2 (&lo)[10]) {
            constexpr bool FUSED = decltype(Fc)::value;
            constexpr int R = decltype(Rc)::value;
            if (y) lk_vmcnt0();
            if (y + 1 < kWin) dma_union(std::integral_constant<int, 1 - R>{}, y + 1);
            if (y + 2 <= kWin) dma_j(Rc, y + 2);
            __builtin_amdgcn_sched_barrier(0);
            uint32_t rj[11];
            read_j(std::integral_constant<int, 1 - R>{}, rj);
            lds_u2v* lE = (lds_u2v*)(ubuf(Rc) + el);
            v2u dcs[10];
#pragma unroll
            for (int gi = 0; gi < 10; gi++) dcs[gi] = lE[4 * gi];
#pragma unroll
            for (int gi = 0; gi < 10; gi++) {
                const v2u dc = dcs[gi];
                lo[gi] = __builtin_bit_cast(s2, __builtin_amdgcn_perm(rj[gi + 1], rj[gi], sel));
                const int jd = __builtin_amdgcn_sdot2(up[gi], W0, __builtin_amdgcn_sdot2(lo[gi], W1, (int)dc.y, false),
                                                      false) >> 9;
                const float fd = (float)jd;
                const f2 f = {(float)(int16_t)dc.x, (float)((int)dc.x >> 16)};
                if constexpr (FUSED) acc = lk_fma(f, fd, acc);
                else acc = acc + f * fd;
            }
            asm volatile("" : "+v"(acc));
        };
        const bool fused = a.fma && __all(!act || certd);
        if (a.body_cnt) (fused ? n_fused : n_exact)++;
        if (fused) {
#pragma unroll 1
            for (int y = 0; y < kWin; y += 2) {
                row(std::true_type{}, y, I0{}, pa, pb);
                row(std::true_type{}, y + 1, I1{}, pb, pa);
            }
        } else {
#pragma unroll 1
            for (int y = 0; y < kWin; y += 2) {
                row(std::false_type{}, y, I0{}, pa, pb);
                row(std::false_type{}, y + 1, I1{}, pb, pa);
            }
        }
        if (!act) acc = f2{0.f, 0.f};
        const float b1s = (quad_bcast<0>(acc.x) + quad_bcast<2>(acc.x)) + (quad_bcast<1>(acc.x) + quad_bcast<3>(acc.x));
        const float b2s = (quad_bcast<0>(acc.y) + quad_bcast<2>(acc.y)) + (quad_bcast<1>(acc.y) + quad_bcast<3>(acc.y));
        if (act) {
            const float b1 = b1s * FLT_SCALE, b2 = b2s * FLT_SCALE;
            const float dx = (A12 * b2 - A22 * b1) * Dinv;
            const float dy = (A12 * b1 - A11 * b2) * Dinv;
            if (a.dbg && pt == a.dbg_pt && pair == 0) {
                float4* t = a.dbg + (long long)a.g.nlev * a.npts + (level * 16 + j) * 4;
                if (k == 0) { t[0] = make_float4(b1s, b2s, dx, dy); t[1] = make_float4(nx, ny, A11, Dinv); }
                t[2 + (k >> 1)] = make_float4(k & 1 ? 0.f : acc.x, k & 1 ? 0.f : acc.y, acc.x, acc.y);
            }
            nx = nx + dx;
            ny = ny + dy;
            npx = nx + HALFW;
            npy = ny + HALFW;
            if ((double)dx * dx + (double)dy * dy <= a.eps2) {
                act = false;
            } else if (j > 0 && fabs((double)fabsf(dx + pdx)) < 0.01 && fabs((double)fabsf(dy + pdy)) < 0.01) {
                npx = npx - dx * 0.5f;
                npy = npy - dy * 0.5f;
                act = false;
            }
            pdx = dx;
            pdy = dy;
        }
        if (live) {
            j++;
            if ((__ballot(act) & smask) == 0 || j >= a.max_iters) {
                live = false;
                retire();
            }
        }
    }
    if (a.body_cnt && lane == 0) {
        atomicAdd(a.body_cnt + 2 * level, n_exact);
        atomicAdd(a.body_cnt + 2 * level + 1, n_fused);
    }
    if (a.dbg && lane == 0 && blockIdx.x < kLkDbgWaves) {
        uint4* st = reinterpret_cast<uint4*>(a.dbg + (long long)batch * a.g.nlev * a.npts + kLkDbgStampOff) +
                    (long long)level * kLkDbgWaves + blockIdx.x;
        const unsigned long long t_end = __builtin_amdgcn_s_memrealtime();
        *st = make_uint4((uint32_t)t_start, (uint32_t)(t_start >> 32), (uint32_t)t_end, (uint32_t)(t_end >> 32));
    }
}

__global__ __launch_bounds__(64) void k_lk_gate(const int* __restrict__ qctr, long long T, const int* __restrict__ done,
                                                int dep_groups, int ngroups_next, long long T_next, int* __restrict__ err,
                                                int spin_max, int* __restrict__ giveup)
{
    const int x = threadIdx.x;
    bool ready = true;
    if (x < 8) {
        const long long cb = T * x / 8, ce = T * (x + 1) / 8;
        const long long cbn = T_next * x / 8;
        const int pf = cbn < T_next ? (int)(cbn / ngroups_next) : -1;
        ready = false;
        for (int t = 0; t < spin_max; t++) {
            const bool dry = __hip_atomic_load(qctr + x * kCtrPad, __ATOMIC_RELAXED, __HIP_MEMORY_SCOPE_AGENT) >= ce - cb;
            const bool first = pf < 0 || __hip_atomic_load(done + pf * kCtrPad, __ATOMIC_RELAXED,
                                                           __HIP_MEMORY_SCOPE_AGENT) >= dep_groups;
            if (dry && first) {
                ready = true;
                break;
            }
            __builtin_amdgcn_s_sleep(8);
        }
    }
    if (!__all(ready) && x == 0) {
        __hip_atomic_fetch_add(err + 1, 1, __ATOMIC_RELAXED, __HIP_MEMORY_SCOPE_AGENT);
        __hip_atomic_fetch_add(giveup, 1, __ATOMIC_RELAXED, __HIP_MEMORY_SCOPE_AGENT);
    }
}

template <int G, int UW, bool DF>
static int lk_iter_resident()
{
    constexpr int kDevs = 64;
    static std::atomic<int> cached[kDevs];
    int dev = 0;
    (void)hipGetDevice(&dev);
    int v = dev >= 0 && dev < kDevs ? cached[dev].load(std::memory_order_relaxed) : 0;
    if (!v) {
        int ncu = 0, nb = 0;
        (void)hipDeviceGetAttribute(&ncu, hipDeviceAttributeMultiprocessorCount, dev);
        (void)hipOccupancyMaxActiveBlocksPerMultiprocessor(&nb, k_lk_iter<G, UW, DF>, 64, 0);
        v = std::max(1, ncu) * std::max(1, nb);
        if (dev >= 0 && dev < kDevs) cached[dev].store(v, std::memory_order_relaxed);
    }
    return v;
}

static int lk_groups(const ClassPlan& plan, int l, int nyg) { return (plan.lv[l].nxp / plan.lv[l].G) * nyg; }

template <int G, int UW>
static void launch_A(hipStream_t s, int batch, const LkArgs& a, const uint8_t* cls, float4* Ab, uint8_t* cert, int* qctr,
                     int l)
{
    constexpr int S = LkShape<G, UW>::S;
    const int ngroups = lk_groups(a.plan, l, a.nyg);
    const dim3 grid((ngroups + S - 1) / S, batch);
    hipLaunchKernelGGL((k_lk_A<G, UW>), grid, dim3(64), 0, s, a, cls, Ab, cert, qctr, l, ngroups);
}

template <int G, int UW>
static void launch_A_rows(hipStream_t s, int batch, const LkArgs& a, const uint8_t* cls, float4* Ab, uint8_t* cert,
                          int* qctr, int l)
{
    constexpr int S = LkShape<G, UW>::S;
    const ClassLevel& C = a.plan.lv[l];
    const int ncg = C.nxp / G;
    const dim3 grid(((ncg + S - 1) / S) * C.nstrip, batch);
    if (C.asp >= 10)
        hipLaunchKernelGGL((k_lk_A_rows<G, UW, 4>), grid, dim3(64), 0, s, a, cls, Ab, cert, qctr, l, ncg);
    else
        hipLaunchKernelGGL((k_lk_A_rows<G, UW, 8>), grid, dim3(64), 0, s, a, cls, Ab, cert, qctr, l, ncg);
}

template <int G, int UW>
static void launch_iter(hipStream_t s, int batch, const LkArgs& a, const uint8_t* cls, const float4* Ab,
                        const uint8_t* cert, int* qctr, int l)
{
    constexpr int S = LkShape<G, UW>::S;
    const int ngroups = lk_groups(a.plan, l, a.nyg);
    const int need = (int)std::min<long long>(((long long)batch * ngroups + S - 1) / S, 1 << 30);
    const bool df = a.done || a.redo || a.lflags || a.dep_groups;
    int res = df ? lk_iter_resident<G, UW, true>() : lk_iter_resident<G, UW, false>();
    if (a.done) res = res * std::min(std::max(a.flow_cap, 10), 100) / 100;
    int W = std::max(8, std::min((need + 7) / 8, res / 8) * 8);
    if (a.redo) W = std::max(8, std::min(W, kLkRedoWaves));
    if (df)
        hipLaunchKernelGGL((k_lk_iter<G, UW, true>), dim3(W), dim3(64), 0, s, a, cls, Ab, cert, qctr, l, ngroups, batch);
    else
        hipLaunchKernelGGL((k_lk_iter<G, UW, false>), dim3(W), dim3(64), 0, s, a, cls, Ab, cert, qctr, l, ngroups, batch);
}

static bool launch_level(bool iter, hipStream_t st, int batch, const LkArgs& a, const uint8_t* cls, float4* Ab,
                         uint8_t* cert, int* qctr, int l)
{
    const ClassLevel& C = a.plan.lv[l];
    switch (C.G * 1000 + C.UW) {
#define LK_CASE(g, uw)                                                   \
    case g * 1000 + uw:                                                  \
        if (iter) launch_iter<g, uw>(st, batch, a, cls, Ab, cert, qctr, l);    \
        else if (C.asp) launch_A_rows<g, uw>(st, batch, a, cls, Ab, cert, qctr, l); \
        else launch_A<g, uw>(st, batch, a, cls, Ab, cert, qctr, l);            \
        return true;
        LK_SHAPES
#undef LK_CASE
    default: return false;
    }
}

static hipError_t lk_enqueue_planes(const LkLaunch& L, hipStream_t sa, int batch, int p, int nb, const LkArgs& a,
                                    const LkArgs& b, uint8_t* bcls, int* bq)
{
    if (L.aux) {
        hipEvent_t ready = L.prev_ready;
        if (!ready || p) {
            if (hipError_t e = hipEventRecord(L.ev[kMaxLevels], L.s)) return e;
            ready = L.ev[kMaxLevels];
        }
        if (hipError_t e = hipStreamWaitEvent(sa, ready, 0)) return e;
    }
    for (int l = a.maxl; l >= 0; l--) {
        const ClassLevel& C = a.plan.lv[l];
        if (L.aux && L.lvl_done) {
            if (hipError_t e = hipStreamWaitEvent(sa, L.lvl_done[l], 0)) return e;
        }
        LkClassArgs ca;
        ca.g = a.g;
        ca.plan = a.plan;
        ca.rlist = a.rlist;
        ca.level = l;
        if (C.nrx * C.nry <= 4) {
            const dim3 grid(((a.g.lv[l].w + 2 * kPad) / 4 + 63) / 64, C.vhi - C.vlo, nb);
            hipLaunchKernelGGL(k_lk_class_fused, grid, dim3(64), 0, sa, b.pyr1, bcls, ca);
        } else {
            const dim3 grid(((a.g.lv[l].w + 2 * kPad) / 4 + 63) / 64, C.vhi - C.vlo, nb * C.nrx * C.nry);
            if (hipError_t e = launch_scharr(sa, nb, b.pyr1, const_cast<uint32_t*>(b.der), a.g, l, C.vlo, C.vhi + 1))
                return e;
            hipLaunchKernelGGL(k_lk_class, grid, dim3(64), 0, sa, b.pyr1, b.der, bcls, ca);
        }
        float4* bA = L.Ab + ((long long)l * batch + p) * a.npts;
        uint8_t* bC = L.cert + ((long long)l * batch + p) * a.npts;
        if (!launch_level(false, sa, nb, b, bcls, bA, bC, bq, l)) return hipErrorInvalidValue;
        if (L.aux) {
            if (hipError_t e = hipEventRecord(L.ev[l], sa)) return e;
        }
    }
    return hipSuccess;
}

static hipError_t lk_enqueue_iters(const LkLaunch& L, int batch, int p, int nb, const LkArgs& a, const LkArgs& b,
                                   uint8_t* bcls, int* bq)
{
    const bool flow_ok = L.aux && L.s2 && L.flow_ev && L.done && L.redo_ev && a.err && b.carry &&
                         (reinterpret_cast<uintptr_t>(b.carry) & 127) == 0 && (a.carry_lstride % 32) == 0;
    const bool flow = flow_ok && nb % 8 == 0 && nb >= 16 && a.npts % 16 == 0 &&
                      (reinterpret_cast<uintptr_t>(b.next_pts) & 127) == 0;
    int* lflags = flow ? L.done + (long long)kMaxLevels * nb * kCtrPad : nullptr;
    if (flow) {
        if (hipError_t e = hipMemsetAsync(L.done, 0, sizeof(int) * ((long long)kMaxLevels * nb + kLkFlagInts) * kCtrPad, L.s))
            return e;
        if (hipError_t e = hipEventRecord(L.flow_ev[0], L.s)) return e;
        if (hipError_t e = hipStreamWaitEvent(L.s2, L.flow_ev[0], 0)) return e;
    }
    for (int l = a.maxl; l >= 0; l--) {
        hipStream_t st = flow && ((a.maxl - l) & 1) ? L.s2 : L.s;
        if (L.aux) {
            if (hipError_t e = hipStreamWaitEvent(st, L.ev[l], 0)) return e;
        }
        LkArgs bl = b;
        bl.done = flow ? L.done : nullptr;
        bl.done_stride = nb;
        bl.dep_groups = 0;
        bl.lflags = lflags;
        bl.redo = 0;
        if (flow && l < a.maxl) {
            const int ngc = lk_groups(a.plan, l + 1, a.nyg), ng = lk_groups(a.plan, l, a.nyg);
            bl.dep_groups = ngc;
            hipLaunchKernelGGL(k_lk_gate, dim3(1), dim3(64), 0, st, bq + (l + 1) * 8 * kCtrPad, (long long)nb * ngc,
                               L.done + (l + 1) * nb * kCtrPad, bl.dep_groups, ng, (long long)nb * ng, a.err,
                               a.spin_max, lflags + (kLkFlagGiveup + l) * kCtrPad);
        }
        float4* bA = L.Ab + ((long long)l * batch + p) * a.npts;
        uint8_t* bC = L.cert + ((long long)l * batch + p) * a.npts;
        if (!launch_level(true, st, nb, bl, bcls, bA, bC, bq, l)) return hipErrorInvalidValue;
        if (flow) {
            if (l < a.maxl) {
                if (hipError_t e = hipStreamWaitEvent(st, L.redo_ev[l + 1], 0)) return e;
                LkArgs br = bl;
                br.done = nullptr;
                br.dep_groups = 0;
                br.redo = 1;
                br.dbg = nullptr;
                br.body_cnt = nullptr;
                if (!launch_level(true, st, nb, br, bcls, bA, bC, bq, l)) return hipErrorInvalidValue;
            }
            if (hipError_t e = hipEventRecord(L.redo_ev[l], st)) return e;
        }
        if (L.lvl_done) {
            if (hipError_t e = hipEventRecord(L.lvl_done[l], st)) return e;
        }
    }
    if (flow) {
        if (hipError_t e = hipEventRecord(L.flow_ev[1], L.s2)) return e;
        if (hipError_t e = hipStreamWaitEvent(L.s, L.flow_ev[1], 0)) return e;
    }
    return hipSuccess;
}

hipError_t launch_lk_v2(const LkLaunch& L, int batch, const LkArgs& a)
{
    const long long span = std::max(a.plan.bytes_per_pair, a.g.img_bytes);
    int sub = batch;
    while (sub > 1 && ((sub + 7) / 8 + 1) * span > 0x7fff0000LL) sub = std::max(1, sub / 2);
    if (a.max_sub > 0) sub = std::max(1, std::min(sub, a.max_sub));
    hipStream_t sa = L.aux ? L.aux : L.s;
    for (int p = 0, si = 0; p < batch; p += sub, si++) {
        const int nb = std::min(sub, batch - p);
        LkArgs b = a;
        b.pyr1 = a.pyr1 + (long long)p * a.g.img_bytes;
        b.pyr2 = a.pyr2 + (long long)p * a.g.img_bytes;
        b.der = a.der + (long long)p * a.g.der_words;
        b.next_pts = a.next_pts + (long long)p * a.npts * 2;
        b.carry = a.carry ? a.carry + (long long)p * a.npts * 2 : nullptr;
        b.status = a.status + (long long)p * a.npts;
        if (p) b.dbg = nullptr;
        uint8_t* bcls = L.cls + (long long)p * a.plan.bytes_per_pair;
        int* bq = L.qctr + si * kMaxLevels * 8 * kCtrPad;
        if (hipError_t e = lk_enqueue_planes(L, sa, batch, p, nb, a, b, bcls, bq)) return e;
        if (hipError_t e = lk_enqueue_iters(L, batch, p, nb, a, b, bcls, bq)) return e;
    }
    return hipGetLastError();
}

}
```

motion_detection_amd/csrc/mdx_pair.cpp:

```cpp
#include "mdx_ctx.h"

#include <cmath>
#include <cstdlib>

using namespace mdx;

static int ensure_class_plan(mdx_ctx* c, const Geometry& g, int w, int h, int ps, int batch, int gy0, int gy1)
{
    int rc;
    const std::array<int, 6> key = {w, h, ps, g.nlev, gy0, gy1};
    if (c->plan_key != key) {
        const int nx = (w + ps - 1) / ps, ny = (h + ps - 1) / ps;
        static_assert(kMaxLevels <= 8, "residue tables sized for 2^7 residues");
        std::vector<int16_t> tab(2 * kMaxLevels * 2 * 128, (int16_t)-1);
        std::vector<int16_t> ord;
        int16_t* cmap = tab.data();
        int16_t* rlist = tab.data() + kMaxLevels * 2 * 128;
        ClassPlan P{};
        bool usable = true;
        for (int l = 0; l < g.nlev; l++) {
            const int m = (1 << l) - 1;
            int n[2] = {0, 0};
            for (int axis = 0; axis < 2; axis++) {
                const int cnt = axis == 0 ? nx : ny;
                for (int i = 0; i < cnt; i++) {
                    const int r = (i * ps) & m;
                    int16_t& slot = cmap[(l * 2 + axis) * 128 + r];
                    if (slot < 0) {
                        slot = (int16_t)n[axis];
                        rlist[(l * 2 + axis) * 128 + n[axis]] = (int16_t)r;
                        n[axis]++;
                    }
                    if (n[axis] == m + 1) break;
                }
            }
            ClassLevel& C = P.lv[l];
            C.nrx = n[0];
            C.nry = n[1];
            C.ord_off = (int)ord.size();
            const int16_t* cmx = cmap + (l * 2 + 0) * 128;
            auto ipx_of = [&](int gx) { return lk_win_origin(gx, ps, l); };
            std::vector<std::vector<int16_t>> runs(n[0]);
            for (int i = 0; i < nx; i++) runs[cmx[(i * ps) & m]].push_back((int16_t)i);
            auto union_of = [&](int G) {
                int u = 0;
                for (const auto& r : runs)
                    for (size_t q = 0; q < r.size(); q += G)
                        u = std::max(u, ipx_of(r[std::min(r.size(), q + G) - 1]) - ipx_of(r[q]) + kWin);
                return u;
            };
            const int u4 = union_of(4), u8 = union_of(8);
            auto fit = [](const int* uws, int n, int u) {
                for (int i = 0; i < n; i++)
                    if (uws[i] >= u) return uws[i];
                return 0;
            };
            const int uw4 = fit(kLkUW4, (int)(sizeof(kLkUW4) / sizeof(int)), u4);
            const int uw8 = fit(kLkUW8, (int)(sizeof(kLkUW8) / sizeof(int)), u8);
            auto pieces = [](int slots, int uw) { return (slots * uw * 8 + 1023) / 1024; };
            const bool g4 = c->lk_g == 4 ? uw4 > 0
                          : c->lk_g == 8 ? false
                          : uw4 > 0 && (uw8 == 0 || pieces(4, uw4) <= pieces(2, uw8));
            if (g4) {
                C.G = 4;
                C.UW = uw4;
            } else {
                C.G = 8;
                C.UW = uw8;
            }
            if (C.UW == 0) usable = false;
            for (const auto& r : runs) {
                ord.insert(ord.end(), r.begin(), r.end());
                for (size_t q = r.size(); q % C.G; q++) ord.push_back((int16_t)-1);
            }
            C.nxp = (int)ord.size() - C.ord_off;
            const size_t r0 = ord.size();
            for (int i = gy0; i < gy1; i++) ord.push_back((int16_t)i);
            const int16_t* cmy = cmap + (l * 2 + 1) * 128;
            std::stable_sort(ord.begin() + r0, ord.end(),
                             [&](int16_t u, int16_t v) { return cmy[(u * ps) & m] < cmy[(v * ps) & m]; });
            const size_t r1 = ord.size();
            auto v0_row = [&](int gy) { return lk_win_origin(gy, ps, l) + kPad; };
            int asp = 0;
            bool uniform = true;
            std::vector<int16_t> strips;
            for (size_t i = r0; i < r1;) {
                size_t e = i + 1;
                const int cls = cmy[(ord[i] * ps) & m];
                while (e < r1 && cmy[(ord[e] * ps) & m] == cls) {
                    const int d = v0_row(ord[e]) - v0_row(ord[e - 1]);
                    if (asp == 0) asp = d;
                    if (d != asp) uniform = false;
                    e++;
                }
                const size_t srows = c->lk_astrip > 0 ? (size_t)c->lk_astrip
                                                      : (size_t)(c->max_batch <= 4 ? 4 : kAStripRows);
                for (size_t s = i; s < e; s += srows) {
                    strips.push_back((int16_t)(s - r0));
                    strips.push_back((int16_t)std::min<size_t>(srows, e - s));
                }
                i = e;
            }
            if (asp == 0) asp = kWin;
            C.asp = uniform && asp >= 5 ? asp : 0;
            C.nstrip = (int)strips.size() / 2;
            C.strip_off = (int)ord.size();
            ord.insert(ord.end(), strips.begin(), strips.end());
        }
        (void)ny;
        long long off = 0;
        for (int l = 0; l < g.nlev; l++) {
            ClassLevel& C = P.lv[l];
            C.UH = g.lv[l].h + 79;
            C.PW = (g.lv[l].w + kPad + std::max(C.UW, 64) + 3) & ~3;
            C.vlo = lk_win_row0(lk_win_origin(gy0, ps, l), C.UH);
            C.vhi = lk_win_row0(lk_win_origin(gy1 - 1, ps, l), C.UH) + kWin;
            C.class_bytes = (long long)C.UH * C.PW * 8;
            C.off = off;
            off += (long long)C.nrx * C.nry * C.class_bytes;
        }
        if (off > 0x7fff0000LL) usable = false;
        P.nch = usable ? 1 : 0;
        P.bytes_per_pair = (off + 255) / 256 * 256;
        tab.insert(tab.end(), ord.begin(), ord.end());
        if ((rc = ensure(c, c->ctab, tab.size() * sizeof(int16_t))) != MDX_OK) return rc;
        HIP_OR_RETURN(c, hipStreamSynchronize(c->stream));
        HIP_OR_RETURN(c, hipMemcpy(c->ctab.p, tab.data(), tab.size() * sizeof(int16_t), hipMemcpyHostToDevice));
        c->plan = P;
        c->plan_key = key;
    }
    if (c->plan.nch == 0) return MDX_OK;
    if ((rc = ensure(c, c->cls, (size_t)c->plan.bytes_per_pair * batch + 64)) != MDX_OK) return rc;
    return MDX_OK;
}

static int wait_input(mdx_ctx* c, hipStream_t st)
{
    if (!c->input_ev) return MDX_OK;
    hipEvent_t e = c->input_ev;
    c->input_ev = nullptr;
    HIP_OR_RETURN(c, hipStreamWaitEvent(st, e, 0));
    return MDX_OK;
}

static inline void mark(mdx_ctx* c, int i, hipStream_t st = nullptr)
{
    if (!c->timing || c->ev.empty()) return;
    if (i == 0) {
        c->cur = c->ncalls < (int)c->ev.size() / 7 ? c->ncalls : -1;
        c->ncalls++;
    }
    if (c->cur >= 0) (void)hipEventRecord(c->ev[c->cur * 7 + i], st ? st : c->stream);
}

struct LkScratch {
    size_t qctr, done, carry, carry_level, cert, bytes;
};
static LkScratch lk_scratch(int nlev, int batch, int npts)
{
    LkScratch s;
    s.qctr = (size_t)nlev * batch * npts * sizeof(float4);
    s.done = s.qctr + (size_t)batch * kMaxLevels * 8 * kCtrPad * sizeof(int);
    s.carry = s.done + ((size_t)kMaxLevels * batch + kLkFlagInts) * kCtrPad * sizeof(int);
    s.carry_level = ((size_t)batch * npts * 8 + 127) / 128 * 128;
    s.cert = s.carry + s.carry_level * nlev;
    s.bytes = s.cert + (size_t)nlev * batch * npts;
    return s;
}

int mdx::run_lk(mdx_ctx* c, const Geometry& g, LkArgs& a, int batch, int w, int h, int gy0, int gy1, bool have_scharr,
                hipEvent_t prev_ready)
{
    int rc;
    hipStream_t s = c->stream;
    bool v2 = c->lk_impl == 2 && a.prev_pts == nullptr;
    if (v2) {
        if ((rc = ensure_class_plan(c, g, w, h, c->prm.pixel_step, batch, gy0, gy1)) != MDX_OK) return rc;
        v2 = c->plan.nch != 0;
    }
    if (!v2) {
        if (gy0 != 0 || gy1 != a.ny)
            return set_err(c, MDX_EINVAL, "row bands need the class-plane LK (pixel_step too large)");
        if (!have_scharr) HIP_OR_RETURN(c, launch_scharr_levels(s, batch, a.pyr1, const_cast<uint32_t*>(a.der), g));
        HIP_OR_RETURN(c, launch_lk(s, batch, a));
        return MDX_OK;
    }
    a.plan = c->plan;
    a.max_sub = c->lk_sub;
    a.err = c->errw.as<int>();
    a.spin_max = c->spin_max;
    a.flow_cap = c->lk_cap;
    a.fma = c->lk_fma ? 1 : 0;
    a.cmap = c->ctab.as<int16_t>();
    a.rlist = c->ctab.as<int16_t>() + kMaxLevels * 2 * 128;
    a.ord = c->ctab.as<int16_t>() + 2 * kMaxLevels * 2 * 128;
    const int npts = a.npts;
    if (c->lk_debug) {
        if ((rc = ensure(c, c->dbg, ((size_t)npts * g.nlev * batch + kLkDbgStampOff + kMaxLevels * kLkDbgWaves) * 16)) !=
            MDX_OK)
            return rc;
        a.dbg = c->dbg.as<float4>();
        const char* e = std::getenv("MDX_LK_DEBUG_PT");
        a.dbg_pt = e ? std::atoi(e) : -1;
        if ((rc = ensure(c, c->lkcnt, kMaxLevels * 2 * sizeof(uint32_t))) != MDX_OK) return rc;
        HIP_OR_RETURN(c, hipMemsetAsync(c->lkcnt.p, 0, kMaxLevels * 2 * sizeof(uint32_t), s));
        a.body_cnt = c->lkcnt.as<uint32_t>();
    }
    const LkScratch sc = lk_scratch(g.nlev, batch, npts);
    if ((rc = ensure(c, c->Abuf, sc.bytes)) != MDX_OK) return rc;
    const std::array<size_t, 4> lay = {reinterpret_cast<size_t>(c->Abuf.p), (size_t)g.nlev, (size_t)batch, (size_t)npts};
    if (c->lk_scratch_key != lay) {
        HIP_OR_RETURN(c, hipStreamSynchronize(c->stream));
        c->lk_scratch_key = lay;
    }
    uint8_t* base = c->Abuf.as<uint8_t>();
    a.carry = reinterpret_cast<float*>(base + sc.carry);
    a.carry_lstride = (long long)(sc.carry_level / sizeof(float));
    LkLaunch L = c->lk;
    L.cls = c->cls.as<uint8_t>();
    L.Ab = c->Abuf.as<float4>();
    L.cert = base + sc.cert;
    L.qctr = reinterpret_cast<int*>(base + sc.qctr);
    L.done = reinterpret_cast<int*>(base + sc.done);
    L.lvl_done = c->prm.call_pipelining ? c->lvl_done : nullptr;
    L.prev_ready = prev_ready;
    HIP_OR_RETURN(c, launch_lk_v2(L, batch, a));
    return MDX_OK;
}

static void band_rows(const Geometry& g, const ClassPlan& P, RowSpan* rows)
{
    for (int l = g.nlev - 1; l >= 0; l--) {
        const int h = g.lv[l].h;
        const int lo = P.lv[l].vlo - 1 - kPad, hi = P.lv[l].vhi + 2 - kPad;
        int clo = std::max(lo, 0), chi = std::min(hi, h);
        if (lo < 0) chi = std::max(chi, std::min(h, 1 - lo));
        if (hi > h) clo = std::min(clo, std::max(0, 2 * h - 1 - hi));
        if (l + 1 < g.nlev) {
            clo = std::min(clo, std::max(0, 2 * rows[l + 1].lo - 2));
            chi = std::max(chi, std::min(h, 2 * rows[l + 1].hi + 2));
        }
        rows[l] = RowSpan{clo, std::max(clo, chi)};
    }
}

static int run_warp_diff(mdx_ctx* c, int batch, const WarpArgs& a)
{
    const size_t wsb = warp_scratch_bytes(batch, a.w, (a.row1 < 0 ? a.h : a.row1) - a.row0);
    if (const int rc = ensure(c, c->wscr, wsb); rc != MDX_OK) return rc;
    HIP_OR_RETURN(c, launch_warp_diff(c->stream, batch, a, c->wscr.p, wsb, &c->last_warp));
    return MDX_OK;
}
static GrayPlane pyr_gray(uint8_t* slab, const Geometry& g)
{
    return {level0_core(slab, g), g.img_bytes, g.lv[0].pitch};
}

struct PipelineArgs {
    int batch;
    const uint8_t *d_img1, *d_img2;
    int w, h, stride;
    size_t frame_stride;
    int fmt;
    float* d_np;
    uint8_t* d_st;
    double* d_vec = nullptr;
    uint8_t* d_mask = nullptr;
    double* d_H = nullptr;
    int* d_num = nullptr;
    const double* d_Hext = nullptr;
    int gy0 = 0, gy1 = -1;
    mdx_band_cand* cand = nullptr;
    bool may_overlap = false;
};
static int run_pipeline(mdx_ctx* c, const PipelineArgs& A)
{
    const mdx_params& P = c->prm;
    const int batch = A.batch, w = A.w, h = A.h, stride = A.stride, fmt = A.fmt;
    mdx_band_cand* const cand = A.cand;
    if (w <= 0 || h <= 0 || batch <= 0) return set_err(c, MDX_EINVAL, "bad frame size or batch");
    int rc = check_frame(c, nullptr, w, h, stride, fmt);
    if (rc != MDX_OK) return rc;
    if (batch > 1 && A.frame_stride < (size_t)stride * h) return set_err(c, MDX_EINVAL, "frame_stride too small");
    if (P.fit_mode == MDX_FIT_EXTERNAL && !A.d_Hext) return set_err(c, MDX_EINVAL, "fit_mode EXTERNAL needs H_external");
    HIP_OR_RETURN(c, hipSetDevice(c->device));
    const bool pipe = A.may_overlap && P.call_pipelining && c->aux && c->lk_impl == 2;
    Geometry g = make_geometry(w, h, P.max_level);
    if ((rc = ensure_workspace(c, g, batch, pipe)) != MDX_OK) return rc;
    const int npts = mdx_grid_count(w, h, P.pixel_step);
    const int ny = (h + P.pixel_step - 1) / P.pixel_step;
    const int gy0 = A.gy0, gy1 = A.gy1 < 0 ? ny : A.gy1;
    const int nyb = gy1 - gy0;
    hipStream_t s = c->stream;
    uint8_t* pyr1 = c->pyr1.as<uint8_t>();
    uint8_t* pyr2 = c->pyr2.as<uint8_t>();
    uint32_t* der = c->der.as<uint32_t>();
    PairFit* fits = c->fits.as<PairFit>();
    hipStream_t fs_ = s;
    int half = 0;
    if (pipe) {
        half = c->pyr_half;
        c->pyr_half ^= 1;
        pyr1 += half * pyr_half_bytes(c->pyr1);
        pyr2 += half * pyr_half_bytes(c->pyr2);
        fs_ = c->aux;
        HIP_OR_RETURN(c, hipStreamWaitEvent(fs_, c->pyr_free[half], 0));
    }
    if ((rc = wait_input(c, fs_)) != MDX_OK) return rc;
    c->last_pyr1 = pyr1;
    c->last_pyr2 = pyr2;
    if (cand) {
        c->band_pyr1 = pyr1;
        c->band_pyr2 = pyr2;
        c->band_half = half;
    } else {
        c->band_w = c->band_h = 0;
    }

    mark(c, 0, fs_);
    hipEvent_t prev_ready = nullptr;
    const uint8_t *d_img1 = A.d_img1, *d_img2 = A.d_img2;
    const long long fs = (long long)A.frame_stride;
    RowSpan rows[kMaxLevels];
    const RowSpan* prows = nullptr;
    if (cand && c->lk_impl == 2 && npts > 0 && nyb > 0 && nyb < ny) {
        if ((rc = ensure_class_plan(c, g, w, h, P.pixel_step, batch, gy0, gy1)) != MDX_OK) return rc;
        if (c->plan.nch != 0) {
            band_rows(g, c->plan, rows);
            prows = rows;
        }
    }
    c->band_built[0] = 0;
    c->band_built[1] = h;
    if (prows) {
        const int lo1 = std::min(rows[1].lo, rows[0].lo / 2), hi1 = std::max(rows[1].hi, (rows[0].hi + 1) / 2);
        c->band_built[0] = std::max(0, 2 * lo1);
        c->band_built[1] = std::min(h, 2 * hi1);
    }
    if (c->aux && c->lk_impl == 2) {
        HIP_OR_RETURN(c, launch_front(fs_, batch, d_img1, d_img2, w, h, stride, fs, fmt, pyr1, pyr2, g, 1, prows));
        mark(c, 1, fs_);
        HIP_OR_RETURN(c, launch_pyr_levels(fs_, batch, pyr1, pyr2, g, 1, prows));
        HIP_OR_RETURN(c, hipEventRecord(c->lkev[kMaxLevels + 1], fs_));
        prev_ready = c->lkev[kMaxLevels + 1];
        HIP_OR_RETURN(c, launch_front(fs_, batch, d_img1, d_img2, w, h, stride, fs, fmt, pyr1, pyr2, g, 2));
        HIP_OR_RETURN(c, launch_pyr_levels(fs_, batch, pyr1, pyr2, g, 2));
        if (pipe) {
            mark(c, 2, fs_);
            HIP_OR_RETURN(c, hipEventRecord(c->front_ev, fs_));
            HIP_OR_RETURN(c, hipStreamWaitEvent(s, c->front_ev, 0));
        }
    } else {
        HIP_OR_RETURN(c, launch_front(s, batch, d_img1, d_img2, w, h, stride, fs, fmt, pyr1, pyr2, g));
        mark(c, 1);
        HIP_OR_RETURN(c, launch_pyr_levels(s, batch, pyr1, pyr2, g));
    }
    if (!pipe) mark(c, 2);
    mark(c, 3);
    if (npts > 0 && nyb > 0) {
        LkArgs a = lk_args_for(c, g, w, h);
        a.pyr1 = pyr1;
        a.pyr2 = pyr2;
        a.der = der;
        a.nyg = nyb;
        a.next_pts = A.d_np;
        a.status = A.d_st;
        if ((rc = run_lk(c, g, a, batch, w, h, gy0, gy1, false, prev_ready)) != MDX_OK) return rc;
    }
    mark(c, 4);
    if ((rc = ensure(c, c->csum, classify_scratch_bytes(batch, npts))) != MDX_OK) return rc;
    FitArgs fa = {A.d_np, A.d_st, npts, ny, P.pixel_step, gy0, gy1, P.min_vector_size, A.d_vec, fits, P.fit_mode,
                  A.d_Hext, c->csum.p, cand, RansacArgs{}};
    if (P.fit_mode == MDX_FIT_RANSAC && !cand) {
        if ((rc = ensure(c, c->rsc, ransac_scratch_bytes(batch, npts, P.ransac_iters))) != MDX_OK) return rc;
        fa.ransac = ransac_args(c->rsc.p, batch, npts, P);
    }
    HIP_OR_RETURN(c, launch_classify_fit(s, batch, fa));
    mark(c, 5);
    if (A.d_mask && !cand) {
        const WarpArgs wa = {pyr_gray(pyr1, g), pyr_gray(pyr2, g), w, h, fits, A.d_mask, (long long)w * h, P.thresh};
        if ((rc = run_warp_diff(c, batch, wa)) != MDX_OK) return rc;
    }
    if ((A.d_H || A.d_num) && !cand) HIP_OR_RETURN(c, launch_export_fit(s, batch, fits, A.d_H, A.d_num));
    if (pipe) HIP_OR_RETURN(c, hipEventRecord(c->pyr_free[half], s));
    else release_pyr_all(c);
    mark(c, 6);
    return MDX_OK;
}

extern "C" int mdx_flow_warp_diff_batch_dev(mdx_ctx* c, int batch, const uint8_t* d_img1, const uint8_t* d_img2,
                                            int w, int h, int stride, size_t frame_stride, int fmt, float* d_next_pts,
                                            uint8_t* d_status, double* d_vectors, uint8_t* d_mask, double* d_H,
                                            const double* d_H_external, int* d_num_vectors)
{
    if (!c) return MDX_EINVAL;
    if (!d_img1 || !d_img2 || batch <= 0) return set_err(c, MDX_EINVAL, "null frame pointer or batch <= 0");
    HIP_OR_RETURN(c, hipSetDevice(c->device));
    const size_t need = (size_t)mdx_grid_count(w, h, c->prm.pixel_step) * batch;
    int rc;
    if (!d_next_pts) {
        if ((rc = ensure(c, c->bnp, need * 8)) != MDX_OK) return rc;
        d_next_pts = c->bnp.as<float>();
    }
    if (!d_status) {
        if ((rc = ensure(c, c->bst, need)) != MDX_OK) return rc;
        d_status = c->bst.as<uint8_t>();
    }
    PipelineArgs A = {batch, d_img1, d_img2, w, h, stride, frame_stride, fmt, d_next_pts, d_status,
                      d_vectors, d_mask, d_H, d_num_vectors, d_H_external};
    A.may_overlap = true;
    return run_pipeline(c, A);
}

extern "C" int mdx_flow_warp_diff(mdx_ctx* c, const uint8_t* img1, const uint8_t* img2, int w, int h, int stride,
                                  int fmt, float* next_pts, uint8_t* status, double* vectors, uint8_t* mask, double* H,
                                  const double* H_external, int* num_vectors)
{
    if (!c) return MDX_EINVAL;
    if (!img1 || !img2) return set_err(c, MDX_EINVAL, "null frame pointer");
    int rc = check_frame(c, nullptr, w, h, stride, fmt);
    if (rc != MDX_OK) return rc;
    if (c->prm.fit_mode == MDX_FIT_EXTERNAL && !H_external)
        return set_err(c, MDX_EINVAL, "fit_mode EXTERNAL needs H_external");
    HIP_OR_RETURN(c, hipSetDevice(c->device));
    const size_t in_bytes = (size_t)stride * h;
    const size_t copy_bytes = frame_copy_bytes(w, h, stride, fmt);
    const int npts = mdx_grid_count(w, h, c->prm.pixel_step);
    const size_t pts = (size_t)(npts > 0 ? npts : 1);
    if ((rc = ensure_all(c, {{&c->in1, in_bytes}, {&c->in2, in_bytes}, {&c->np, pts * 8}, {&c->st, pts},
                             {&c->vec, pts * 32}, {&c->mask, (size_t)w * h}, {&c->H, 72}, {&c->Hext, 72},
                             {&c->num, 4}})) != MDX_OK)
        return rc;

    hipStream_t s = c->stream;
    HIP_OR_RETURN(c, hipMemcpyAsync(c->in1.p, img1, copy_bytes, hipMemcpyHostToDevice, s));
    HIP_OR_RETURN(c, hipMemcpyAsync(c->in2.p, img2, copy_bytes, hipMemcpyHostToDevice, s));
    if (H_external) HIP_OR_RETURN(c, hipMemcpyAsync(c->Hext.p, H_external, 72, hipMemcpyHostToDevice, s));
    const PipelineArgs A = {1, c->in1.as<uint8_t>(), c->in2.as<uint8_t>(), w, h, stride, in_bytes, fmt, c->np.as<float>(),
                            c->st.as<uint8_t>(), vectors ? c->vec.as<double>() : nullptr,
                            mask ? c->mask.as<uint8_t>() : nullptr, c->H.as<double>(), c->num.as<int>(),
                            H_external ? c->Hext.as<double>() : nullptr};
    if ((rc = run_pipeline(c, A)) != MDX_OK) return rc;
    int num = 0;
    if (next_pts && npts > 0) HIP_OR_RETURN(c, hipMemcpyAsync(next_pts, c->np.p, (size_t)npts * 8, hipMemcpyDeviceToHost, s));
    if (status && npts > 0) HIP_OR_RETURN(c, hipMemcpyAsync(status, c->st.p, (size_t)npts, hipMemcpyDeviceToHost, s));
    if (vectors && npts > 0) HIP_OR_RETURN(c, hipMemcpyAsync(vectors, c->vec.p, (size_t)npts * 32, hipMemcpyDeviceToHost, s));
    if (mask) HIP_OR_RETURN(c, hipMemcpyAsync(mask, c->mask.p, (size_t)w * h, hipMemcpyDeviceToHost, s));
    if (H) HIP_OR_RETURN(c, hipMemcpyAsync(H, c->H.p, 72, hipMemcpyDeviceToHost, s));
    HIP_OR_RETURN(c, hipMemcpyAsync(&num, c->num.p, 4, hipMemcpyDeviceToHost, s));
    HIP_OR_RETURN(c, hipStreamSynchronize(s));
    if (num_vectors) *num_vectors = num;
    if (c->prm.fit_mode != MDX_FIT_EXTERNAL && num < 4) return MDX_EDEGENERATE;
    return MDX_OK;
}

extern "C" int mdx_warp_diff_dev(mdx_ctx* c, int batch, const uint8_t* d_gray1, const uint8_t* d_gray2, int w, int h,
                                 int stride, size_t frame_stride, const double* d_H, uint8_t* d_mask)
{
    if (!c) return MDX_EINVAL;
    if (!d_gray1 || !d_gray2 || !d_H || !d_mask || batch <= 0 || w <= 0 || h <= 0 || stride < w)
        return set_err(c, MDX_EINVAL, "mdx_warp_diff_dev: bad argument");
    HIP_OR_RETURN(c, hipSetDevice(c->device));
    int rc = ensure(c, c->fits, sizeof(PairFit) * (size_t)batch);
    if (rc != MDX_OK) return rc;
    hipStream_t s = c->stream;
    PairFit* fits = c->fits.as<PairFit>();
    if ((rc = wait_input(c, s)) != MDX_OK) return rc;
    for (int i = 0; i < 5; i++) mark(c, i);
    HIP_OR_RETURN(c, launch_set_fit_external(s, batch, d_H, fits));
    mark(c, 5);
    const long long fs = (long long)frame_stride;
    const WarpArgs wa = {{d_gray1, fs, stride}, {d_gray2, fs, stride}, w, h, fits, d_mask, (long long)w * h, c->prm.thresh};
    if ((rc = run_warp_diff(c, batch, wa)) != MDX_OK) return rc;
    mark(c, 6);
    return MDX_OK;
}

extern "C" int mdx_probe_stream3_dev(mdx_ctx* c, size_t n, const uint8_t* d_a, const uint8_t* d_b, uint8_t* d_mask,
                                     int thresh)
{
    if (!c) return MDX_EINVAL;
    if (!d_a || !d_b || !d_mask || n == 0 || n % 16 || ((uintptr_t)d_a | (uintptr_t)d_b | (uintptr_t)d_mask) % 16)
        return set_err(c, MDX_EINVAL, "mdx_probe_stream3_dev: bad argument");
    HIP_OR_RETURN(c, hipSetDevice(c->device));
    for (int i = 0; i < 6; i++) mark(c, i);
    HIP_OR_RETURN(c, launch_stream3(c->stream, n, d_a, d_b, d_mask, thresh));
    mark(c, 6);
    return MDX_OK;
}

extern "C" int mdx_band_flow_dev(mdx_ctx* c, const uint8_t* d_img1, const uint8_t* d_img2, int w, int h, int stride,
                                 int fmt, int y0, int y1, float* d_next_pts, uint8_t* d_status, double* d_vectors,
                                 mdx_band_cand* d_cand)
{
    if (!c) return MDX_EINVAL;
    if (!d_img1 || !d_img2 || !d_next_pts || !d_status || !d_cand)
        return set_err(c, MDX_EINVAL, "mdx_band_flow_dev: null pointer");
    if (w <= 0 || h <= 0 || y0 < 0 || y1 > h || y0 >= y1) return set_err(c, MDX_EINVAL, "bad band [%d, %d) of %d rows", y0, y1, h);
    if (c->prm.fit_mode != MDX_FIT_FIRST4) return set_err(c, MDX_EINVAL, "row bands need fit_mode FIRST4");
    const int ps = c->prm.pixel_step;
    const int gy0 = (y0 + ps - 1) / ps, gy1 = (y1 + ps - 1) / ps;
    c->band_w = c->band_h = 0;
    PipelineArgs A = {1, d_img1, d_img2, w, h, stride, (size_t)stride * h, fmt, d_next_pts, d_status, d_vectors};
    A.gy0 = gy0;
    A.gy1 = gy1;
    A.cand = d_cand;
    A.may_overlap = true;
    const int rc = run_pipeline(c, A);
    if (rc == MDX_OK) {
        c->band_w = w;
        c->band_h = h;
        c->band_img1 = d_img1;
        c->band_stride = stride;
        c->band_fmt = fmt;
    }
    return rc;
}

extern "C" int mdx_band_fit_warp_dev(mdx_ctx* c, int nrec, const mdx_band_cand* d_cands, int y0, int y1,
                                     uint8_t* d_mask_band, double* d_H, int* d_num_vectors)
{
    if (!c) return MDX_EINVAL;
    if (nrec <= 0 || !d_cands || !d_mask_band) return set_err(c, MDX_EINVAL, "mdx_band_fit_warp_dev: bad argument");
    const int w = c->band_w, h = c->band_h;
    if (w <= 0 || h <= 0)
        return set_err(c, MDX_EINVAL, "mdx_band_fit_warp_dev: no mdx_band_flow_dev before, or another call rebuilt "
                                      "the context's pyramids since");
    if (y0 < 0 || y1 > h || y0 >= y1) return set_err(c, MDX_EINVAL, "bad band [%d, %d) of %d rows", y0, y1, h);
    HIP_OR_RETURN(c, hipSetDevice(c->device));
    const Geometry g = make_geometry(w, h, c->prm.max_level);
    hipStream_t s = c->stream;
    PairFit* fits = c->fits.as<PairFit>();
    if (!c->band_pyr1 || !c->band_img1) return set_err(c, MDX_EINVAL, "mdx_band_fit_warp_dev: no mdx_band_flow_dev before");
    HIP_OR_RETURN(c, launch_band_fit(s, nrec, d_cands, fits, w, h, y0, y1));
    HIP_OR_RETURN(c, launch_gray_rows(s, c->band_img1, w, h, c->band_stride, c->band_fmt,
                                      level0_core(c->band_pyr1, g), g.lv[0].pitch, fits, c->band_built[0],
                                      c->band_built[1]));
    const WarpArgs wa = {pyr_gray(c->band_pyr1, g), pyr_gray(c->band_pyr2, g), w, h, fits, d_mask_band,
                         (long long)w * (y1 - y0), c->prm.thresh, y0, y1};
    if (const int rc = run_warp_diff(c, 1, wa); rc != MDX_OK) return rc;
    if (d_H || d_num_vectors) HIP_OR_RETURN(c, launch_export_fit(s, 1, fits, d_H, d_num_vectors));
    if (c->prm.call_pipelining) HIP_OR_RETURN(c, hipEventRecord(c->pyr_free[c->band_half], s));
    else release_pyr_all(c);
    return MDX_OK;
}
```

Measured before the change: 8679.

## Precompute per-run exactness flags in class kernels and load them in LK A-pass

The class-plane kernels now compute, per 32-column run, a conservative flag saying whether any derivative-intensity product could exceed the exact-float range, and store it in a new summary buffer. The A-matrix kernels then replace the per-pixel magnitude max tracking with one byte load per window row from that summary and OR the flags together. This removes per-element abs/max ALU work from the hot A accumulation loop. In exchange it adds extra work and stores in the class kernels, extra scratch memory, an added outstanding load per row in the A pipeline, and a coarser, more conservative certification that may fail more points. A debug readback for the cert buffer is also added.

```diff
diff --git a/motion_detection_amd/csrc/mdx_api.cpp b/motion_detection_amd/csrc/mdx_api.cpp
--- a/motion_detection_amd/csrc/mdx_api.cpp
+++ b/motion_detection_amd/csrc/mdx_api.cpp
@@ -275,6 +275,15 @@
         return MDX_OK;
     }
 #endif
+    if (which == 9) {
+        if (!c->last_cert) return set_err(c, MDX_EINVAL, "debug buffer %d unavailable", which);
+        HIP_OR_RETURN(c, hipStreamSynchronize(c->stream));
+        const size_t n = (size_t)c->last_cert_npts;
+        const size_t rows = std::min((size_t)c->last_cert_nlev, bytes / n);
+        if (rows)
+            HIP_OR_RETURN(c, hipMemcpy2D(dst, n, c->last_cert, n * c->last_cert_batch, n, rows, hipMemcpyDeviceToHost));
+        return MDX_OK;
+    }
     DevBuf& b = which == 0 ? c->Abuf : which == 1 ? c->dbg : which == 2 ? c->pyr1 : which == 3 ? c->pyr2
               : which == 4 ? c->der : which == 6 ? c->lkcnt : which == 7 ? c->sdata : which == 8 ? c->scnt : c->cls;
     if (!b.p) return set_err(c, MDX_EINVAL, "debug buffer %d unavailable", which);
diff --git a/motion_detection_amd/csrc/mdx_ctx.h b/motion_detection_amd/csrc/mdx_ctx.h
--- a/motion_detection_amd/csrc/mdx_ctx.h
+++ b/motion_detection_amd/csrc/mdx_ctx.h
@@ -91,6 +91,8 @@
     DevBuf cls, Abuf, ctab;
     DevBuf dbg;
     DevBuf lkcnt;
+    const uint8_t* last_cert = nullptr;
+    int last_cert_nlev = 0, last_cert_batch = 0, last_cert_npts = 0;
     DevBuf csum;
     DevBuf tin, tcur, tnp, tst, ttraj, tnum, tflag;
     DevBuf straj, sdata, sq, scnt, scols, sres, sout, sbest;
@@ -117,6 +119,7 @@
     std::array<int, 6> plan_key{{-1, -1, -1, -1, -1, -1}};
     int band_w = 0, band_h = 0;
     mdx::ClassPlan plan{};
+    mdx::CertPlan cert_plan{};
     bool timing = false;
     std::vector<hipEvent_t> ev;
     int ncalls = 0;
diff --git a/motion_detection_amd/csrc/mdx_internal.h b/motion_detection_amd/csrc/mdx_internal.h
--- a/motion_detection_amd/csrc/mdx_internal.h
+++ b/motion_detection_amd/csrc/mdx_internal.h
@@ -56,6 +56,16 @@
     int nstrip;
     int strip_off;
 };
+
+constexpr int kLkRunCols = 32;
+struct CertLevel {
+    int SR;
+    long long off;
+};
+struct CertPlan {
+    CertLevel lv[kMaxLevels];
+    long long bytes_per_pair;
+};
 constexpr int kAStripRows = 16;
 
 __host__ __device__ inline int lk_win_origin(int gi, int pixel_step, int level)
@@ -78,6 +88,7 @@
 struct LkClassArgs {
     Geometry g;
     ClassPlan plan;
+    CertPlan sum;
     const int16_t* rlist;
     int level;
 };
@@ -190,6 +201,8 @@
     uint8_t* cls = nullptr;
     float4* Ab = nullptr;
     uint8_t* cert = nullptr;
+    uint8_t* csum = nullptr;
+    CertPlan sum{};
     int* qctr = nullptr;
     int* done = nullptr;
     hipEvent_t* lvl_done = nullptr;
diff --git a/motion_detection_amd/csrc/mdx_lk.hip b/motion_detection_amd/csrc/mdx_lk.hip
--- a/motion_detection_amd/csrc/mdx_lk.hip
+++ b/motion_detection_amd/csrc/mdx_lk.hip
@@ -128,8 +128,73 @@
     __builtin_nontemporal_store(__builtin_bit_cast(v4nt, b), reinterpret_cast<v4nt*>(o) + 1);
 }
 
+constexpr int kLkT32Max = 8160;
+constexpr uint32_t kLkProdLimit = 1u << 24;
+static_assert(((16385LL * 255 + 256) >> 9) == kLkT32Max, "largest descaled bilinear sum");
+static_assert(4080LL * kLkT32Max < (1LL << 31) && kLkT32Max < (1 << 23), "v_mul_i32_i24 operands and product");
+static_assert(kLkRunCols == 8 * 4, "a run is the 4 columns of each of 8 consecutive lanes");
+struct LkCertAcc {
+    int hi = 0, lo = 0;
+    __device__ __forceinline__ void add(int ixv, int iyv, int ival)
+    {
+        const int bound = max(ival, kLkT32Max - ival);
+        const int px = __mul24(ixv, bound), py = __mul24(iyv, bound);
+        hi = max(hi, max(px, py));
+        lo = min(lo, min(px, py));
+    }
+    __device__ __forceinline__ void add_stored(uint32_t d, int c) { add((int)(int16_t)d, (int)d >> 16, (256 - c) >> 9); }
+    __device__ __forceinline__ void add_pixel(uint32_t d, int i) { add((int)(int16_t)d, (int)d >> 16, 32 * i); }
+    __device__ __forceinline__ bool bad() const { return max(hi, -lo) >= (int)kLkProdLimit; }
+};
+constexpr int kLkMagFree = 2056;
+static_assert((long long)kLkMagFree * kLkT32Max < (1LL << 24), "screened magnitudes cannot fail");
+struct LkMagRange {
+    s2 hi = {0, 0}, lo = {0, 0};
+    __device__ __forceinline__ void add(uint32_t d)
+    {
+        const s2 v = __builtin_bit_cast(s2, d);
+        hi = __builtin_elementwise_max(hi, v);
+        lo = __builtin_elementwise_min(lo, v);
+    }
+    __device__ __forceinline__ bool strong() const
+    {
+        return max(max((int)hi.x, (int)hi.y), -min((int)lo.x, (int)lo.y)) > kLkMagFree;
+    }
+};
+__device__ __forceinline__ bool lk_cert_bad4(const uint32_t (&dv)[4], const int (&cv)[4], const uint32_t (&pd)[4],
+                                             const int (&pi)[4])
+{
+    LkMagRange m;
+    static_for<0, 4>([&](auto qc) {
+        constexpr int q = decltype(qc)::value;
+        m.add(dv[q]);
+        m.add(pd[q]);
+    });
+    bool bad = false;
+    if (__any(m.strong())) {
+        LkCertAcc ca;
+        static_for<0, 4>([&](auto qc) {
+            constexpr int q = decltype(qc)::value;
+            ca.add_stored(dv[q], cv[q]);
+            ca.add_pixel(pd[q], pi[q]);
+        });
+        bad = ca.bad();
+    }
+    return bad;
+}
+__device__ __forceinline__ uint8_t* lk_sum_row(uint8_t* csum, const CertPlan& S, int level, int pair, int cls, int UH, int v)
+{
+    return csum + (long long)pair * S.bytes_per_pair + S.lv[level].off + ((long long)cls * UH + v) * S.lv[level].SR;
+}
+__device__ __forceinline__ void lk_run_store(uint8_t* srow, int j, bool any_bad)
+{
+    const unsigned long long bad = __ballot(any_bad);
+    const int lane = threadIdx.x & 63;
+    if ((lane & 7) == 0) srow[j >> 3] = (uint8_t)(((bad >> lane) & 0xffull) != 0);
+}
+
 __global__ __launch_bounds__(256) void k_lk_class(const uint8_t* __restrict__ pyr1, const uint32_t* __restrict__ der,
-                                                  uint8_t* __restrict__ cls_out, LkClassArgs a)
+                                                  uint8_t* __restrict__ cls_out, uint8_t* __restrict__ csum, LkClassArgs a)
 {
     const int level = a.level;
     const ClassLevel& C = a.plan.lv[level];
@@ -152,6 +217,8 @@
     uint8_t* base = cls_out + (long long)pair * a.plan.bytes_per_pair + C.off + (long long)cls * C.class_bytes;
     uint32_t dv[4] = {0, 0, 0, 0};
     int cv[4];
+    uint32_t pd[4] = {0, 0, 0, 0};
+    int pi[4] = {0, 0, 0, 0};
     const int x0 = 4 * j - kPad;
     if (y < L.h + kPad - 1 && x0 < L.w + kPad - 1) {
         const uint8_t* ip = I + (long long)y * p + x0;
@@ -175,18 +242,26 @@
             dv[q] = ((uint32_t)ixv & 0xffffu) | ((uint32_t)iyv << 16);
             cv[q] = 256 - 512 * ival;
         });
+        static_for<0, 4>([&](auto qc) {
+            constexpr int q = decltype(qc)::value;
+            if (x0 + q < L.w + kPad - 1) {
+                pd[q] = dw[0][q];
+                pi[q] = (int)((ib[0][0] >> (8 * q)) & 255u);
+            }
+        });
     } else {
 #pragma unroll
         for (int q = 0; q < 4; q++) cv[q] = 256;
     }
     uint4* o = reinterpret_cast<uint4*>(base) + ((long long)v * C.PW + 4 * j) / 2;
     cls_store(o, dv, cv);
+    lk_run_store(lk_sum_row(csum, a.sum, level, pair, cls, C.UH, v), j, lk_cert_bad4(dv, cv, pd, pi));
 }
 
 __device__ __forceinline__ int u8_at(const uint32_t (&w)[3], int b) { return (int)((w[b >> 2] >> (8 * (b & 3))) & 255u); }
 
 __global__ __launch_bounds__(256) void k_lk_class_fused(const uint8_t* __restrict__ pyr1, uint8_t* __restrict__ cls_out,
-                                                        LkClassArgs a)
+                                                        uint8_t* __restrict__ csum, LkClassArgs a)
 {
     const int level = a.level;
     const ClassLevel& C = a.plan.lv[level];
@@ -229,6 +304,16 @@
             }
             dw[r][c] = d;
         }
+    }
+    uint32_t pd[4] = {0, 0, 0, 0};
+    int pi[4] = {0, 0, 0, 0};
+    if (inside) {
+#pragma unroll
+        for (int q = 0; q < 4; q++)
+            if (x0 + q < L.w + kPad - 1) {
+                pd[q] = dw[0][q];
+                pi[q] = u8_at(rw[1], 4 + q);
+            }
     }
     for (int cls = 0; cls < nclass; cls++) {
         const int rx = residue_of(a.rlist, level, 0, cls % C.nrx), ry = residue_of(a.rlist, level, 1, cls / C.nrx);
@@ -253,6 +338,7 @@
         uint8_t* base = cls_out + (long long)pair * a.plan.bytes_per_pair + C.off + (long long)cls * C.class_bytes;
         uint4* o = reinterpret_cast<uint4*>(base) + ((long long)v * C.PW + 4 * j) / 2;
         cls_store(o, dv, cv);
+        lk_run_store(lk_sum_row(csum, a.sum, level, pair, cls, C.UH, v), j, lk_cert_bad4(dv, cv, pd, pi));
     }
 }
 
@@ -275,11 +361,19 @@
     int v0;
     uint32_t ubase;
 };
-
-template <int G, int UW>
-__device__ __forceinline__ GroupGeom group_geom(const LkArgs& a, const ClassLevel& C, int level, int g, int sl)
-{
-    GroupGeom r;
+struct GroupGeomA : GroupGeom {
+    int cls, c0;
+};
+__device__ __forceinline__ int lk_lane_run(int c0, int k)
+{
+    static_assert(kWin <= 2 * kLkRunCols + 1, "a window row touches at most 3 runs, a quad has 4 lanes");
+    return min(c0 / kLkRunCols + k, (c0 + kWin - 1) / kLkRunCols);
+}
+
+template <int G, int UW, typename Geom = GroupGeom>
+__device__ __forceinline__ Geom group_geom(const LkArgs& a, const ClassLevel& C, int level, int g, int sl)
+{
+    Geom r;
     const int16_t* xo = a.ord + C.ord_off;
     const int16_t* yo = xo + C.nxp;
     const bool has = g >= 0;
@@ -301,6 +395,10 @@
     r.off = min(max(r.ipx + kPad - ub, 0), UW - kWin);
     r.v0 = lk_win_row0(r.ipy, C.UH);
     r.ubase = (uint32_t)(C.off + (long long)(cy * C.nrx + cx) * C.class_bytes) + 8u * (uint32_t)ub;
+    if constexpr (std::is_same_v<Geom, GroupGeomA>) {
+        r.cls = cy * C.nrx + cx;
+        r.c0 = ub + r.off;
+    }
     return r;
 }
 
@@ -363,23 +461,38 @@
     return make_float4(A11, A12, A22, Dinv);
 }
 
-constexpr float kLkCertMax = 2056.f;
-static_assert(kLkCertMax * 8160.f < 16777216.f, "certified products are exact in float");
-__device__ __forceinline__ float lk_mag_max(float m, f2 f)
-{
-    return __builtin_fmaxf(__builtin_fmaxf(m, __builtin_fabsf(f.x)), __builtin_fabsf(f.y));
+struct LkSumLevel {
+    const uint8_t* base;
+    long long bytes_per_pair;
+    long long off;
+    int SR;
+};
+struct LkRunFlags {
+    __amdgpu_buffer_rsrc_t rs;
+    uint32_t voff;
+    uint32_t rowb;
+    __device__ __forceinline__ uint32_t load(int t) const
+    {
+        return __builtin_amdgcn_raw_buffer_load_b8(rs, (int)voff, (int)((uint32_t)t * rowb), 0);
+    }
+};
+__device__ __forceinline__ LkRunFlags lk_run_flags(const LkSumLevel& su, int pair, int cls, int UH, int v0, int c0, int k)
+{
+    return LkRunFlags{buf_rsrc(su.base + (long long)pair * su.bytes_per_pair, su.bytes_per_pair),
+                      (uint32_t)(su.off + ((long long)cls * UH + v0) * su.SR) + (uint32_t)lk_lane_run(c0, k),
+                      (uint32_t)su.SR};
 }
 __device__ __forceinline__ f2 lk_fma(f2 f, float fd, f2 acc) { return __builtin_elementwise_fma(f, f2{fd, fd}, acc); }
-__device__ __forceinline__ uint8_t lk_cert_flag(float m)
-{
-    const float q = __builtin_fmaxf(__builtin_fmaxf(quad_bcast<0>(m), quad_bcast<1>(m)),
-                                    __builtin_fmaxf(quad_bcast<2>(m), quad_bcast<3>(m)));
-    return q <= kLkCertMax ? 1 : 0;
+__device__ __forceinline__ uint8_t lk_cert_flag(uint32_t bad)
+{
+    const uint32_t q = (quad_bcast_u<0>(bad) | quad_bcast_u<1>(bad)) | (quad_bcast_u<2>(bad) | quad_bcast_u<3>(bad));
+    return q ? 0 : 1;
 }
 
 template <int G, int UW>
-__global__ __launch_bounds__(64) void k_lk_A(LkArgs a, const uint8_t* __restrict__ cls, float4* __restrict__ Ab,
-                                             uint8_t* __restrict__ cert, int* __restrict__ qctr, int level, int ngroups)
+__global__ __launch_bounds__(64) void k_lk_A(LkArgs a, const uint8_t* __restrict__ cls, LkSumLevel su,
+                                             float4* __restrict__ Ab, uint8_t* __restrict__ cert, int* __restrict__ qctr,
+                                             int level, int ngroups)
 {
     using Sh = LkShape<G, UW>;
     constexpr int LPS = Sh::LPS, S = Sh::S, ND = Sh::ND;
@@ -396,7 +509,7 @@
     const ClassLevel& C = a.plan.lv[level];
     const Level L = a.g.lv[level];
     const int g = w * S + slot;
-    const GroupGeom q = group_geom<G, UW>(a, C, level, g < ngroups ? g : -1, sl);
+    const GroupGeomA q = group_geom<G, UW, GroupGeomA>(a, C, level, g < ngroups ? g : -1, sl);
     bool ok = q.valid && !(q.ipx < -kWin || q.ipx >= L.w || q.ipy < -kWin || q.ipy >= L.h);
 
     LkRowImages<Sh> im{(lds_u32*)img0, (lds_u32*)img1, (lds_u32*)img2,
@@ -406,18 +519,26 @@
     lk_piece_offsets<Sh>(q.ubase + (uint32_t)q.v0 * im.rowb, lane, uoff);
     im.mask_past(lane, uoff);
     const int el = 2 * (slot * UW + q.off + k);
+    const LkRunFlags rf = lk_run_flags(su, pair, q.cls, C.UH, q.v0, q.c0, k);
 
     f2 sd = {0.f, 0.f};
-    float s12 = 0.f, mag = 0.f;
+    float s12 = 0.f;
+    uint32_t bad = 0, fl[NB];
     constexpr int PF = NB - 1;
     im.template dma<0>(uoff);
+    fl[0] = rf.load(0);
     im.template dma<1>(uoff);
+    fl[1] = rf.load(1);
     static_for<0, kWin>([&](auto yc) {
         constexpr int y = decltype(yc)::value;
         constexpr int later = (y + PF - 1 < kWin - 1 ? y + PF - 1 : kWin - 1) - y;
-        lk_vmcnt<later * ND>();
-        if constexpr (y + PF < kWin) im.template dma<(y + PF) % NB>(uoff);
+        lk_vmcnt<later * (ND + 1)>();
+        if constexpr (y + PF < kWin) {
+            im.template dma<(y + PF) % NB>(uoff);
+            fl[(y + PF) % NB] = rf.load(y + PF);
+        }
         __builtin_amdgcn_sched_barrier(0);
+        bad |= fl[y % NB];
         lds_u2v* lE = (lds_u2v*)(im.template ibuf<y % NB>() + el);
         uint32_t dw[10];
 #pragma unroll
@@ -428,12 +549,11 @@
             const f2 f = {(float)(int16_t)d, (float)((int)d >> 16)};
             sd = __builtin_elementwise_fma(f, f, sd);
             s12 = __builtin_fmaf(f.x, f.y, s12);
-            mag = lk_mag_max(mag, f);
-        }
-        asm volatile("" : "+v"(mag));
+        }
+        asm volatile("" : "+v"(bad));
     });
     const float4 r = lk_A_result(sd, s12, ok, a.min_eig);
-    const uint8_t cf = lk_cert_flag(mag);
+    const uint8_t cf = lk_cert_flag(bad);
     if (q.valid && k == 0) {
         Ab[(long long)pair * a.npts + q.gx * a.ny + q.gy] = r;
         cert[(long long)pair * a.npts + q.gx * a.ny + q.gy] = cf;
@@ -441,7 +561,8 @@
 }
 
 template <int G, int UW, int NW>
-__global__ __launch_bounds__(64) void k_lk_A_rows(LkArgs a, const uint8_t* __restrict__ cls, float4* __restrict__ Ab,
+__global__ __launch_bounds__(64) void k_lk_A_rows(LkArgs a, const uint8_t* __restrict__ cls, LkSumLevel su,
+                                                  float4* __restrict__ Ab,
                                                   uint8_t* __restrict__ cert, int* __restrict__ qctr, int level, int ncg)
 {
     using Sh = LkShape<G, UW>;
@@ -486,15 +607,12 @@
     lk_piece_offsets<Sh>(ubase + (uint32_t)v00 * im.rowb, lane, uoff);
     im.mask_past(lane, uoff);
     const int el = 2 * (slot * UW + off + k);
-
-    static_assert(NW % 2 == 0, "slot pairs");
-    typedef unsigned short us2 __attribute__((ext_vector_type(2)));
+    const LkRunFlags rf = lk_run_flags(su, pair, cy * C.nrx + cx, C.UH, v00, ub + off, k);
+
     f2 sd[NW];
     float s12[NW];
-    us2 magp[NW / 2];
+    uint32_t badm = 0, fl[3];
     int rin[NW], jw[NW];
-#pragma unroll
-    for (int s = 0; s < NW / 2; s++) magp[s] = us2{0, 0};
 #pragma unroll
     for (int s = 0; s < NW; s++) {
         sd[s] = f2{0.f, 0.f};
@@ -503,22 +621,25 @@
         jw[s] = 0;
     }
     int nextj = 0;
-    auto finish = [&](int j, f2 sdv, float s12v, float magv) {
+    auto finish = [&](int j, f2 sdv, float s12v, uint32_t badv) {
         const int gy = yo[r0 + j];
         const int ipy = lk_win_origin(gy, a.pixel_step, level);
         const bool ok = valid && !(ipx < -kWin || ipx >= L.w || ipy < -kWin || ipy >= L.h);
         const float4 r = lk_A_result(sdv, s12v, ok, a.min_eig);
-        const uint8_t cf = lk_cert_flag(magv);
+        const uint8_t cf = lk_cert_flag(badv);
         if (valid && k == 0) {
             Ab[(long long)pair * a.npts + gx * a.ny + gy] = r;
             cert[(long long)pair * a.npts + gx * a.ny + gy] = cf;
         }
     };
     auto row = [&](int t, auto bc) {
-        if (t + 1 < R) lk_vmcnt<ND>();
+        if (t + 1 < R) lk_vmcnt<ND + 1>();
         else lk_vmcnt0();
         constexpr int B = decltype(bc)::value;
-        if (t + 2 < R) im.template dma<(B + 2) % 3>(uoff);
+        if (t + 2 < R) {
+            im.template dma<(B + 2) % 3>(uoff);
+            fl[(B + 2) % 3] = rf.load(t + 2);
+        }
         __builtin_amdgcn_sched_barrier(0);
         lds_u2v* lE = (lds_u2v*)(im.template ibuf<B>() + el);
         uint32_t dw[10];
@@ -527,25 +648,20 @@
         f2 f[10];
 #pragma unroll
         for (int gi = 0; gi < 10; gi++) f[gi] = f2{(float)(int16_t)dw[gi], (float)((int)dw[gi] >> 16)};
-        float rmag = 0.f;
-#pragma unroll
-        for (int gi = 0; gi < 10; gi++) rmag = lk_mag_max(rmag, f[gi]);
         if (nextj < nr && t == nextj * asp) {
             static_for<0, NW>([&](auto sc) {
                 constexpr int s = decltype(sc)::value;
                 if (nextj % NW == s) {
                     sd[s] = f2{0.f, 0.f};
                     s12[s] = 0.f;
-                    magp[s / 2][s & 1] = 0;
+                    badm &= ~(1u << s);
                     rin[s] = 0;
                     jw[s] = nextj;
                 }
             });
             nextj++;
         }
-        const unsigned short ri = (unsigned short)(uint32_t)rmag;
-#pragma unroll
-        for (int s = 0; s < NW / 2; s++) magp[s] = __builtin_elementwise_max(magp[s], us2{ri, ri});
+        badm |= 0u - fl[B];
         static_for<0, NW>([&](auto sc) {
             constexpr int s = decltype(sc)::value;
             if (rin[s] >= 0) {
@@ -555,14 +671,19 @@
                     s12[s] = __builtin_fmaf(f[gi].x, f[gi].y, s12[s]);
                 }
                 if (++rin[s] == kWin) {
-                    finish(jw[s], sd[s], s12[s], (float)magp[s / 2][s & 1]);
+                    finish(jw[s], sd[s], s12[s], badm & (1u << s));
                     rin[s] = -1;
                 }
             }
         });
     };
     im.template dma<0>(uoff);
-    if (R > 1) im.template dma<1>(uoff);
+    fl[0] = rf.load(0);
+    fl[1] = fl[2] = 0;
+    if (R > 1) {
+        im.template dma<1>(uoff);
+        fl[1] = rf.load(1);
+    }
 #pragma unroll 1
     for (int t = 0; t < R; t += 3) {
         row(t, std::integral_constant<int, 0>{});
@@ -945,27 +1066,27 @@
 static int lk_groups(const ClassPlan& plan, int l, int nyg) { return (plan.lv[l].nxp / plan.lv[l].G) * nyg; }
 
 template <int G, int UW>
-static void launch_A(hipStream_t s, int batch, const LkArgs& a, const uint8_t* cls, float4* Ab, uint8_t* cert, int* qctr,
-                     int l)
+static void launch_A(hipStream_t s, int batch, const LkArgs& a, const uint8_t* cls, const LkSumLevel& su, float4* Ab,
+                     uint8_t* cert, int* qctr, int l)
 {
     constexpr int S = LkShape<G, UW>::S;
     const int ngroups = lk_groups(a.plan, l, a.nyg);
     const dim3 grid((ngroups + S - 1) / S, batch);
-    hipLaunchKernelGGL((k_lk_A<G, UW>), grid, dim3(64), 0, s, a, cls, Ab, cert, qctr, l, ngroups);
+    hipLaunchKernelGGL((k_lk_A<G, UW>), grid, dim3(64), 0, s, a, cls, su, Ab, cert, qctr, l, ngroups);
 }
 
 template <int G, int UW>
-static void launch_A_rows(hipStream_t s, int batch, const LkArgs& a, const uint8_t* cls, float4* Ab, uint8_t* cert,
-                          int* qctr, int l)
+static void launch_A_rows(hipStream_t s, int batch, const LkArgs& a, const uint8_t* cls, const LkSumLevel& su, float4* Ab,
+                          uint8_t* cert, int* qctr, int l)
 {
     constexpr int S = LkShape<G, UW>::S;
     const ClassLevel& C = a.plan.lv[l];
     const int ncg = C.nxp / G;
     const dim3 grid(((ncg + S - 1) / S) * C.nstrip, batch);
     if (C.asp >= 10)
-        hipLaunchKernelGGL((k_lk_A_rows<G, UW, 4>), grid, dim3(64), 0, s, a, cls, Ab, cert, qctr, l, ncg);
+        hipLaunchKernelGGL((k_lk_A_rows<G, UW, 4>), grid, dim3(64), 0, s, a, cls, su, Ab, cert, qctr, l, ncg);
     else
-        hipLaunchKernelGGL((k_lk_A_rows<G, UW, 8>), grid, dim3(64), 0, s, a, cls, Ab, cert, qctr, l, ncg);
+        hipLaunchKernelGGL((k_lk_A_rows<G, UW, 8>), grid, dim3(64), 0, s, a, cls, su, Ab, cert, qctr, l, ncg);
 }
 
 template <int G, int UW>
@@ -986,16 +1107,16 @@
         hipLaunchKernelGGL((k_lk_iter<G, UW, false>), dim3(W), dim3(64), 0, s, a, cls, Ab, cert, qctr, l, ngroups, batch);
 }
 
-static bool launch_level(bool iter, hipStream_t st, int batch, const LkArgs& a, const uint8_t* cls, float4* Ab,
-                         uint8_t* cert, int* qctr, int l)
+static bool launch_level(bool iter, hipStream_t st, int batch, const LkArgs& a, const uint8_t* cls, const LkSumLevel& su,
+                         float4* Ab, uint8_t* cert, int* qctr, int l)
 {
     const ClassLevel& C = a.plan.lv[l];
     switch (C.G * 1000 + C.UW) {
 #define LK_CASE(g, uw)                                                   \
     case g * 1000 + uw:                                                  \
         if (iter) launch_iter<g, uw>(st, batch, a, cls, Ab, cert, qctr, l);    \
-        else if (C.asp) launch_A_rows<g, uw>(st, batch, a, cls, Ab, cert, qctr, l); \
-        else launch_A<g, uw>(st, batch, a, cls, Ab, cert, qctr, l);            \
+        else if (C.asp) launch_A_rows<g, uw>(st, batch, a, cls, su, Ab, cert, qctr, l); \
+        else launch_A<g, uw>(st, batch, a, cls, su, Ab, cert, qctr, l);      \
         return true;
         LK_SHAPES
 #undef LK_CASE
@@ -1006,6 +1127,7 @@
 static hipError_t lk_enqueue_planes(const LkLaunch& L, hipStream_t sa, int batch, int p, int nb, const LkArgs& a,
                                     const LkArgs& b, uint8_t* bcls, int* bq)
 {
+    uint8_t* const bsum = L.csum + (long long)p * L.sum.bytes_per_pair;
     if (L.aux) {
         hipEvent_t ready = L.prev_ready;
         if (!ready || p) {
@@ -1022,20 +1144,22 @@
         LkClassArgs ca;
         ca.g = a.g;
         ca.plan = a.plan;
+        ca.sum = L.sum;
         ca.rlist = a.rlist;
         ca.level = l;
         if (C.nrx * C.nry <= 4) {
             const dim3 grid(((a.g.lv[l].w + 2 * kPad) / 4 + 63) / 64, C.vhi - C.vlo, nb);
-            hipLaunchKernelGGL(k_lk_class_fused, grid, dim3(64), 0, sa, b.pyr1, bcls, ca);
+            hipLaunchKernelGGL(k_lk_class_fused, grid, dim3(64), 0, sa, b.pyr1, bcls, bsum, ca);
         } else {
             const dim3 grid(((a.g.lv[l].w + 2 * kPad) / 4 + 63) / 64, C.vhi - C.vlo, nb * C.nrx * C.nry);
             if (hipError_t e = launch_scharr(sa, nb, b.pyr1, const_cast<uint32_t*>(b.der), a.g, l, C.vlo, C.vhi + 1))
                 return e;
-            hipLaunchKernelGGL(k_lk_class, grid, dim3(64), 0, sa, b.pyr1, b.der, bcls, ca);
+            hipLaunchKernelGGL(k_lk_class, grid, dim3(64), 0, sa, b.pyr1, b.der, bcls, bsum, ca);
         }
         float4* bA = L.Ab + ((long long)l * batch + p) * a.npts;
         uint8_t* bC = L.cert + ((long long)l * batch + p) * a.npts;
-        if (!launch_level(false, sa, nb, b, bcls, bA, bC, bq, l)) return hipErrorInvalidValue;
+        const LkSumLevel su{bsum, L.sum.bytes_per_pair, L.sum.lv[l].off, L.sum.lv[l].SR};
+        if (!launch_level(false, sa, nb, b, bcls, su, bA, bC, bq, l)) return hipErrorInvalidValue;
         if (L.aux) {
             if (hipError_t e = hipEventRecord(L.ev[l], sa)) return e;
         }
@@ -1077,7 +1201,7 @@
         }
         float4* bA = L.Ab + ((long long)l * batch + p) * a.npts;
         uint8_t* bC = L.cert + ((long long)l * batch + p) * a.npts;
-        if (!launch_level(true, st, nb, bl, bcls, bA, bC, bq, l)) return hipErrorInvalidValue;
+        if (!launch_level(true, st, nb, bl, bcls, LkSumLevel{}, bA, bC, bq, l)) return hipErrorInvalidValue;
         if (flow) {
             if (l < a.maxl) {
                 if (hipError_t e = hipStreamWaitEvent(st, L.redo_ev[l + 1], 0)) return e;
@@ -1087,7 +1211,7 @@
                 br.redo = 1;
                 br.dbg = nullptr;
                 br.body_cnt = nullptr;
-                if (!launch_level(true, st, nb, br, bcls, bA, bC, bq, l)) return hipErrorInvalidValue;
+                if (!launch_level(true, st, nb, br, bcls, LkSumLevel{}, bA, bC, bq, l)) return hipErrorInvalidValue;
             }
             if (hipError_t e = hipEventRecord(L.redo_ev[l], st)) return e;
         }
diff --git a/motion_detection_amd/csrc/mdx_pair.cpp b/motion_detection_amd/csrc/mdx_pair.cpp
--- a/motion_detection_amd/csrc/mdx_pair.cpp
+++ b/motion_detection_amd/csrc/mdx_pair.cpp
@@ -108,7 +108,7 @@
             ord.insert(ord.end(), strips.begin(), strips.end());
         }
         (void)ny;
-        long long off = 0;
+        long long off = 0, soff = 0;
         for (int l = 0; l < g.nlev; l++) {
             ClassLevel& C = P.lv[l];
             C.UH = g.lv[l].h + 79;
@@ -118,7 +118,12 @@
             C.class_bytes = (long long)C.UH * C.PW * 8;
             C.off = off;
             off += (long long)C.nrx * C.nry * C.class_bytes;
+            CertLevel& S = c->cert_plan.lv[l];
+            S.SR = (C.PW + kLkRunCols - 1) / kLkRunCols;
+            S.off = soff;
+            soff += (long long)C.nrx * C.nry * C.UH * S.SR;
         }
+        c->cert_plan.bytes_per_pair = (soff + 255) / 256 * 256;
         if (off > 0x7fff0000LL) usable = false;
         P.nch = usable ? 1 : 0;
         P.bytes_per_pair = (off + 255) / 256 * 256;
@@ -154,9 +159,9 @@
 }
 
 struct LkScratch {
-    size_t qctr, done, carry, carry_level, cert, bytes;
+    size_t qctr, done, carry, carry_level, cert, csum, bytes;
 };
-static LkScratch lk_scratch(int nlev, int batch, int npts)
+static LkScratch lk_scratch(int nlev, int batch, int npts, long long sum_bytes_per_pair)
 {
     LkScratch s;
     s.qctr = (size_t)nlev * batch * npts * sizeof(float4);
@@ -164,7 +169,8 @@
     s.carry = s.done + ((size_t)kMaxLevels * batch + kLkFlagInts) * kCtrPad * sizeof(int);
     s.carry_level = ((size_t)batch * npts * 8 + 127) / 128 * 128;
     s.cert = s.carry + s.carry_level * nlev;
-    s.bytes = s.cert + (size_t)nlev * batch * npts;
+    s.csum = (s.cert + (size_t)nlev * batch * npts + 255) / 256 * 256;
+    s.bytes = s.csum + (size_t)batch * sum_bytes_per_pair;
     return s;
 }
 
@@ -206,7 +212,7 @@
         HIP_OR_RETURN(c, hipMemsetAsync(c->lkcnt.p, 0, kMaxLevels * 2 * sizeof(uint32_t), s));
         a.body_cnt = c->lkcnt.as<uint32_t>();
     }
-    const LkScratch sc = lk_scratch(g.nlev, batch, npts);
+    const LkScratch sc = lk_scratch(g.nlev, batch, npts, c->cert_plan.bytes_per_pair);
     if ((rc = ensure(c, c->Abuf, sc.bytes)) != MDX_OK) return rc;
     const std::array<size_t, 4> lay = {reinterpret_cast<size_t>(c->Abuf.p), (size_t)g.nlev, (size_t)batch, (size_t)npts};
     if (c->lk_scratch_key != lay) {
@@ -220,6 +226,14 @@
     L.cls = c->cls.as<uint8_t>();
     L.Ab = c->Abuf.as<float4>();
     L.cert = base + sc.cert;
+    L.csum = base + sc.csum;
+    L.sum = c->cert_plan;
+    if (c->lk_debug) {
+        c->last_cert = L.cert;
+        c->last_cert_nlev = g.nlev;
+        c->last_cert_batch = batch;
+        c->last_cert_npts = npts;
+    }
     L.qctr = reinterpret_cast<int*>(base + sc.qctr);
     L.done = reinterpret_cast<int*>(base + sc.done);
     L.lvl_done = c->prm.call_pipelining ? c->lvl_done : nullptr;
```

New measurement: 8680, median of 2. No clear change (+0.0%).
